# mataiyuan/ASD-SLAM

Hardware: AMD Instinct MI355X
Metric: frames/sec end-to-end tracking+LocalBA, KITTI 00 mono @2000 keypoints (higher is better)
Workload: dtype f32

## Files before the change

asd-slam_amd/capi.py:

```python
import ctypes as C
import os

import numpy as np

_HERE = os.path.dirname(os.path.abspath(__file__))


def lib_path():
    return os.environ.get("ASDHIP_LIB") or os.path.join(_HERE, "libasdhip.so")


class AsdError(RuntimeError):
    def __init__(self, code, msg):
        super().__init__(f"libasdhip error {code}: {msg}")
        self.code = code


class asd_config(C.Structure):
    _fields_ = [("n_features", C.c_int32), ("scale_factor", C.c_float), ("n_levels", C.c_int32),
                ("ini_th_fast", C.c_int32), ("min_th_fast", C.c_int32), ("max_width", C.c_int32),
                ("max_height", C.c_int32), ("max_patches", C.c_int32), ("device", C.c_int32)]


KP_DTYPE = np.dtype([("x", np.float32), ("y", np.float32), ("size", np.float32), ("angle", np.float32),
# ... 72 lines not shown
    frac = np.empty((h, w), np.uint16)
    rc = lib.asd_undistort_map(_p(Kf), _p(df), int(w), int(h), _p(xy), _p(frac))
    if rc != 0:
        raise AsdError(rc, "asd_undistort_map: invalid arguments")
    return xy, frac


def bow_score(scoring, v1, v2):
    lib = load_library()
    lib.asd_last_error.restype = C.c_char_p
    i1, x1, i2, x2 = _c(v1[0], np.int32), _c(v1[1], np.float64), _c(v2[0], np.int32), _c(v2[1], np.float64)
    out = C.c_double(0.0)
    rc = lib.asd_bow_score(int(scoring), len(i1), _p(i1), _p(x1), len(i2), _p(i2), _p(x2), C.byref(out))
    if rc != 0:
        raise AsdError(rc, lib.asd_last_error(None).decode())
    return out.value


class AsdHip:

    def __init__(self, n_features=2000, scale_factor=1.2, n_levels=8, ini_th=20, min_th=7,
                 max_width=1241, max_height=376, max_patches=None, device=0):
        self.lib = load_library()
        L = self.lib
        L.asd_last_error.restype = C.c_char_p
        L.asd_version.restype = C.c_char_p
        L.asd_ctx_stream.restype = C.c_void_p
        self.cfg = asd_config(n_features, scale_factor, n_levels, ini_th, min_th, max_width, max_height,
                              max_patches if max_patches is not None else 2 * n_features, device)
        self.ctx = C.c_void_p()
        rc = L.asd_ctx_create(C.byref(self.cfg), C.byref(self.ctx))
        if rc != 0:
            raise AsdError(rc, "asd_ctx_create failed (no usable HIP device? there is no CPU fallback)")
        self.n_levels = n_levels

    def close(self):
        if getattr(self, "ctx", None) is not None and self.ctx:
            self.lib.asd_ctx_destroy(self.ctx)
            self.ctx = None

    def __del__(self):
        try:
            self.close()
        except Exception:
            pass

    def _chk(self, rc):
        if rc != 0:
            raise AsdError(rc, self.lib.asd_last_error(self.ctx).decode())

    def last_error(self):
        return self.lib.asd_last_error(self.ctx).decode()

    def calibration_note(self):
        self.lib.asd_calibration_note.restype = C.c_char_p
        return self.lib.asd_calibration_note(self.ctx).decode()

    def scale_tables(self):
        n = self.n_levels
        s, i, g, ig = (np.zeros(n, np.float32) for _ in range(4))
        f = np.zeros(n, np.int32)
        self._chk(self.lib.asd_get_scale_tables(self.ctx, _p(s), _p(i), _p(g), _p(ig), _p(f)))
        return dict(scale=s, inv_scale=i, sigma2=g, inv_sigma2=ig, features_per_level=f)

    def load_weights(self, layers, eps=1e-5):
        ws = [_c(w, np.float32) for w, _, _ in layers]
        ms = [_c(m, np.float32) for _, m, _ in layers]
        vs = [_c(v, np.float32) for _, _, v in layers]
        arr = lambda xs: (C.c_void_p * 7)(*[x.ctypes.data for x in xs])
        self._keep = (ws, ms, vs)
        self._chk(self.lib.asd_load_weights(self.ctx, arr(ws), arr(ms), arr(vs), C.c_float(eps)))

    def describe(self, patches):
        patches = _c(patches, np.uint8).reshape(-1, 32, 32)
        n = patches.shape[0]
        out = np.empty((n, 128), np.float32)
        self._chk(self.lib.asd_describe(self.ctx, _p(patches), n, _p(out)))
        return out

    def device_alloc(self, nbytes):
        p = C.c_void_p()
        self._chk(self.lib.asd_device_alloc(self.ctx, C.c_uint64(nbytes), C.byref(p)))
        return p

    def host_alloc(self, nbytes):
        p = C.c_void_p()
        self._chk(self.lib.asd_host_alloc(self.ctx, C.c_uint64(nbytes), C.byref(p)))
        return p

    def device_free(self, p):
        self._chk(self.lib.asd_device_free(self.ctx, p))

    def h2d(self, dptr, arr):
        arr = np.ascontiguousarray(arr)
        self._chk(self.lib.asd_memcpy_h2d(self.ctx, dptr, _p(arr), C.c_uint64(arr.nbytes)))

    def d2h(self, arr, dptr):
        self._chk(self.lib.asd_memcpy_d2h(self.ctx, _p(arr), dptr, C.c_uint64(arr.nbytes)))

    def sync(self):
        self._chk(self.lib.asd_sync(self.ctx))

    def describe_timed(self, d_patches, n, d_desc, reps):
        ms = C.c_float()
        self._chk(self.lib.asd_describe_timed(self.ctx, d_patches, n, d_desc, reps, C.byref(ms)))
        return ms.value

    def debug_act6(self, n):
        out = np.empty((n, 64, 128), np.float32)
        self.lib.asd_debug_act6.argtypes = [C.c_void_p, C.c_int, C.c_void_p]
        self._chk(self.lib.asd_debug_act6(self.ctx, n, _p(out)))
        return out

    def describe_device(self, d_patches, n, d_desc):
        self._chk(self.lib.asd_describe_device(self.ctx, d_patches, n, d_desc))

    def last_stage_ms(self, stage):
        ms = C.c_float()
        self._chk(self.lib.asd_last_stage_ms(self.ctx, stage.encode(), C.byref(ms)))
        return ms.value

    def extract(self, image, n_features_override=0):
        image = np.asarray(image, np.uint8)
        if image.strides[1] != 1 or image.strides[0] < image.shape[1]:
            image = _c(image, np.uint8)
        h, w = image.shape
        cap = self.cfg.max_patches
        kps = np.zeros(cap, KP_DTYPE)
        desc = np.empty((cap, 128), np.float32)
        n = C.c_int32()
        self._chk(self.lib.asd_extract(self.ctx, _p(image), w, h, image.strides[0], n_features_override,
                                       _p(kps), _p(desc), C.byref(n)))
        return kps[:n.value].copy(), desc[:n.value].copy()

    def extract_device(self, d_image, w, h, stride, n_features_override=0):
        cap = self.cfg.max_patches
        if not hasattr(self, "_kps_buf"):
            self._kps_buf = np.zeros(cap, KP_DTYPE)
            self._desc_buf = np.empty((cap, 128), np.float32)
        n = C.c_int32()
        self._chk(self.lib.asd_extract_device(self.ctx, d_image, w, h, stride, n_features_override,
                                              _p(self._kps_buf), _p(self._desc_buf), C.byref(n)))
        return self._kps_buf[:n.value], self._desc_buf[:n.value]

    def extract_submit(self, image, w, h, stride, device_resident=True, n_features_override=0):
        self._chk(self.lib.asd_extract_submit(self.ctx, image, int(device_resident), w, h, stride, n_features_override))

    def extract_wait(self, view=False):
        n = C.c_int32()
        if view:
            pk, pd = C.c_void_p(), C.c_void_p()
            self._chk(self.lib.asd_extract_wait_view(self.ctx, C.byref(pk), C.byref(pd), C.byref(n)))
            if n.value == 0:
                return np.zeros(0, KP_DTYPE), np.zeros((0, 128), np.float32)
            kb = (C.c_char * (n.value * KP_DTYPE.itemsize)).from_address(pk.value)
            db = (C.c_float * (n.value * 128)).from_address(pd.value)
            return np.frombuffer(kb, dtype=KP_DTYPE, count=n.value), np.frombuffer(db, dtype=np.float32).reshape(n.value, 128)
        cap = self.cfg.max_patches
        if not hasattr(self, "_kps_buf"):
            self._kps_buf = np.zeros(cap, KP_DTYPE)
            self._desc_buf = np.empty((cap, 128), np.float32)
        self._chk(self.lib.asd_extract_wait(self.ctx, _p(self._kps_buf), _p(self._desc_buf), C.byref(n)))
        return self._kps_buf[:n.value], self._desc_buf[:n.value]

    def extract_last_view(self):
        self.lib.asd_extract_last_view.restype = C.c_uint64
        return int(self.lib.asd_extract_last_view(self.ctx))

    def extract_view_valid(self, view_id):
        self.lib.asd_extract_view_valid.restype = C.c_int32
        return bool(self.lib.asd_extract_view_valid(self.ctx, C.c_uint64(view_id)))

    def extract_hold(self, on=True):
        self._chk(self.lib.asd_extract_hold(self.ctx, int(on)))

    def set_undistortion(self, K, dist, w, h):
        Kf = None if K is None else _c(K, np.float32)
        df = None if dist is None else _c(dist, np.float32)
        self._chk(self.lib.asd_set_undistortion(self.ctx, _p(Kf), _p(df), int(w), int(h)))

    def undistort(self, image, device_resident=False, w=None, h=None, stride=None):
        if device_resident:
            src = image
        else:
            image = np.asarray(image)
            assert image.dtype == np.uint8 and image.ndim == 2 and image.strides[1] == 1
            h, w = image.shape
            stride = image.strides[0]
            src = C.c_void_p(image.ctypes.data)
        out = np.empty((h, w), np.uint8)
        self._chk(self.lib.asd_undistort(self.ctx, src, int(device_resident), int(w), int(h), int(stride), _p(out), int(w)))
        return out

    def profile_enable(self, on=True):
        self._chk(self.lib.asd_profile_enable(self.ctx, int(on)))

    def profile_get(self, layer):
        ms, calls, patches = C.c_double(), C.c_int32(), C.c_int64()
        self._chk(self.lib.asd_profile_get(self.ctx, layer, C.byref(ms), C.byref(calls), C.byref(patches)))
        return ms.value, calls.value, patches.value

    def asdnet_split_mask(self):
        self.lib.asd_asdnet_split_mask.restype = C.c_int32
        return int(self.lib.asd_asdnet_split_mask(self.ctx))

    def asdnet_pieces(self):
        self.lib.asd_asdnet_pieces.restype = C.c_int32
        return int(self.lib.asd_asdnet_pieces(self.ctx))

    def level_size(self, level):
        w, h = C.c_int32(), C.c_int32()
        self._chk(self.lib.asd_get_level_size(self.ctx, level, C.byref(w), C.byref(h)))
        return w.value, h.value

    def level_image(self, level, blurred=False):
        w, h = self.level_size(level)
        out = np.empty((h, w), np.uint8)
        self._chk(self.lib.asd_get_level_image(self.ctx, level, int(blurred), _p(out)))
        return out

    def raw_corners(self, level, cap=200000):
        x, y, r = (np.empty(cap, np.float32) for _ in range(3))
        n = C.c_int32()
        self._chk(self.lib.asd_get_raw_corners(self.ctx, level, cap, _p(x), _p(y), _p(r), C.byref(n)))
        return x[:n.value].copy(), y[:n.value].copy(), r[:n.value].copy()

    def patches(self):
        cap = self.cfg.max_patches
        out = np.empty((cap, 32, 32), np.uint8)
        n = C.c_int32()
        self._chk(self.lib.asd_get_patches(self.ctx, cap, _p(out), C.byref(n)))
        return out[:n.value].copy()

    def frame_set(self, slot, kps, desc, bounds):
        kps = _c(kps, KP_DTYPE)
        d = None if desc is None else _c(desc, np.float32)
        self._chk(self.lib.asd_frame_set(self.ctx, slot, _p(kps), _p(d), len(kps), C.c_float(bounds[0]),
                                         C.c_float(bounds[1]), C.c_float(bounds[2]), C.c_float(bounds[3])))

    def frame_set_from_ctx(self, slot, kps, bounds, src):
        kps = _c(kps, KP_DTYPE)
        self._chk(self.lib.asd_frame_set_from_ctx(self.ctx, slot, _p(kps), len(kps), C.c_float(bounds[0]), C.c_float(bounds[1]),
                                                  C.c_float(bounds[2]), C.c_float(bounds[3]), src.ctx))

    def extract_keep_pyramid(self, on=True):
        self._chk(self.lib.asd_extract_keep_pyramid(self.ctx, int(on)))

    def features_in_area(self, slot, x, y, r, min_level=-1, max_level=-1, cap=8192):
        out = np.empty(cap, np.int32)
        n = C.c_int32()
        self._chk(self.lib.asd_frame_features_in_area(self.ctx, slot, C.c_float(x), C.c_float(y), C.c_float(r),
                                                      min_level, max_level, cap, _p(out), C.byref(n)))
        return out[:n.value].copy()

    def dist_matrix(self, a, b):
        a, b = _c(a, np.float32), _c(b, np.float32)
        out = np.empty((a.shape[0], b.shape[0]), np.float32)
        self._chk(self.lib.asd_dist_matrix(self.ctx, _p(a), a.shape[0], _p(b), b.shape[0], _p(out)))
        return out

    def distinctive_descriptor(self, desc):
        desc = _c(desc, np.float32)
        best = C.c_int32()
        self._chk(self.lib.asd_distinctive_descriptor(self.ctx, _p(desc), desc.shape[0], C.byref(best)))
        return best.value

    def match_project_frame(self, slot_cur, slot_last, n_cur, has_mp, Xw, mp_desc, Tcw, K, th, check_ori=True, obs_positive=None):
        has_mp, Xw, mp_desc = _c(has_mp, np.uint8), _c(Xw, np.float32), _c(mp_desc, np.float32)
        Tcw, K = _c(Tcw, np.float32), _c(K, np.float32)
        out = np.empty(n_cur, np.int32)
        n = C.c_int32()
        self._chk(self.lib.asd_match_project_frame(self.ctx, slot_cur, slot_last, _p(has_mp), _p(Xw), _p(mp_desc),
                                                   _p(Tcw), _p(K), C.c_float(th), int(check_ori), _p(out),
                                                   C.byref(n), _p(None if obs_positive is None else _c(obs_positive, np.uint8))))
        return out, n.value

    def match_project_points(self, slot_cur, n_cur, in_view, proj, level, view_cos, desc, occupied, th, nn_ratio, obs_positive=None):
        in_view, proj, level = _c(in_view, np.uint8), _c(proj, np.float32), _c(level, np.int32)
        view_cos, desc, occupied = _c(view_cos, np.float32), _c(desc, np.float32), _c(occupied, np.uint8)
        out = np.empty(n_cur, np.int32)
        n = C.c_int32()
        self._chk(self.lib.asd_match_project_points(self.ctx, slot_cur, len(in_view), _p(in_view), _p(proj),
                                                    _p(level), _p(view_cos), _p(desc), _p(occupied), C.c_float(th),
                                                    C.c_float(nn_ratio), _p(out), C.byref(n),
                                                    _p(None if obs_positive is None else _c(obs_positive, np.uint8))))
        return out, n.value

    def track_motion_model(self, slot_cur, slot_last, n_cur, has_mp, Xw, mp_desc_or_rows, Tcw, K, th, pose7, check_ori=True, obs_positive=None, split=False):
        has_mp, Xw, Tcw, K = _c(has_mp, np.uint8), _c(Xw, np.float32), _c(Tcw, np.float32), _c(K, np.float32)
        d = np.asarray(mp_desc_or_rows)
        bank = d.dtype.kind in "iu"
        d = _c(d, np.int32 if bank else np.float32)
        match, outl = np.empty(n_cur, np.int32), np.empty(max(n_cur, 1), np.uint8)
        pose = _c(pose7, np.float64).copy()
        n, ninl = C.c_int32(), C.c_int32()
        fn = self.lib.asd_track_motion_model_bank if bank else self.lib.asd_track_motion_model
        if split:
            self._chk(self.lib.asd_track_async(self.ctx))
        self._chk(fn(self.ctx, slot_cur, slot_last, _p(has_mp), _p(Xw), _p(d), _p(Tcw), _p(K), C.c_float(th), int(check_ori),
                     _p(None if obs_positive is None else _c(obs_positive, np.uint8)), _p(pose), _p(match), C.byref(n), _p(outl), C.byref(ninl)))
        if split:
            self._track_job = (match, n, pose, outl, ninl, n_cur)
            return None
        return match, n.value, pose, outl[:n_cur], ninl.value

    def track_local_map(self, slot_cur, n_cur, in_view, proj, level, view_cos, desc_or_rows, mp_Xw, occupied, cur_Xw, th, nn_ratio, K, pose7,
                        obs_positive=None, split=False):
        in_view, proj, level = _c(in_view, np.uint8), _c(proj, np.float32), _c(level, np.int32)
        view_cos, mp_Xw, occupied, cur_Xw, K = _c(view_cos, np.float32), _c(mp_Xw, np.float32), _c(occupied, np.uint8), _c(cur_Xw, np.float32), _c(K, np.float32)
        d = np.asarray(desc_or_rows)
        bank = d.dtype.kind in "iu"
        d = _c(d, np.int32 if bank else np.float32)
        match, outl = np.empty(n_cur, np.int32), np.empty(max(n_cur, 1), np.uint8)
        pose = _c(pose7, np.float64).copy()
        n, ninl = C.c_int32(), C.c_int32()
        fn = self.lib.asd_track_local_map_bank if bank else self.lib.asd_track_local_map
# ... 475 lines not shown
```

asd-slam_amd/csrc/asdnet.hip:

```cpp
#include "ctx.h"

#include <algorithm>
#include <cmath>
#include <cstring>

typedef float f32x16 __attribute__((ext_vector_type(16)));
typedef float f32x4 __attribute__((ext_vector_type(4)));


namespace {

struct LayerSpec { int cout, cin, k, stride, pad; };
const LayerSpec kLayers[7] = {{32, 1, 3, 1, 1},   {32, 32, 3, 1, 1},   {64, 32, 3, 2, 1},  {64, 64, 3, 1, 1},
                              {128, 64, 3, 2, 1}, {128, 128, 3, 1, 1}, {128, 128, 8, 1, 0}};

template <int CIN, int COUT, int HIN, int S, int ROWS, int WM, int WN, int KC, int PP = 1, int RING = 2>
struct ConvCfg {
  static constexpr int HO = HIN / S;
  static constexpr int INROWS = (ROWS - 1) * S + 3;
  static constexpr int INCOLS = (HO - 1) * S + 3;
  static constexpr int CPAD = CIN + 4;
  static constexpr int NW = WM * WN;
  static constexpr int NTH = 64 * NW;
  static constexpr int M_PATCH = ROWS * HO;
// ... 1180 lines not shown
  const _Float16 hh = (_Float16)xs;
  const _Float16 ll = (_Float16)(xs - (float)hh);
  memcpy(&h, &hh, 2);
  memcpy(&l, &ll, 2);
}

inline float weight_scale_f16(const float* w, size_t count, const std::vector<float>& inv, size_t per_cout) {
  float mx = 0.f;
  for (size_t i = 0; i < count; ++i) mx = std::max(mx, std::fabs(w[i] * inv[i / per_cout]));
  if (!(mx > 0.f) || !std::isfinite(mx)) return 1.f;
  int e;
  (void)std::frexp(mx, &e);
  return std::ldexp(1.f, 14 - e);
}

void build_wx3(const LayerSpec& L, const float* w, const std::vector<float>& inv, std::vector<uint16_t>& img, int np = 3, float wscale = 1.f) {
  img.assign((size_t)9 * L.cin * L.cout * np, 0);
  constexpr int kch = 32, kg = kch / 8;
  const int nc16 = L.cin / kch;
  for (int tap = 0; tap < 9; ++tap)
    for (int ci = 0; ci < L.cin; ++ci)
      for (int co = 0; co < L.cout; ++co) {
        const float v = w[((size_t)co * L.cin + ci) * 9 + tap] * inv[co];
        uint16_t p[3];
        if (np == 3) split3_host(v, p[0], p[1], p[2]);
        else split2_host(v * wscale, p[0], p[1]);
        const int c16 = ci / kch, hh = (ci % kch) / 8, j = ci % 8;
        for (int q = 0; q < np; ++q)
          img[(((((size_t)tap * nc16 + c16) * np + q) * kg + hh) * L.cout + co) * 8 + j] = p[q];
      }
}

void build_wimg(const LayerSpec& L, const float* w, const std::vector<float>& inv, std::vector<float>& img) {
  img.assign((size_t)9 * L.cin * L.cout, 0.f);
  for (int tap = 0; tap < 9; ++tap)
    for (int ci = 0; ci < L.cin; ++ci)
      for (int co = 0; co < L.cout; ++co) {
        const int c8 = ci / 8, hh = (ci % 8) / 4, jj = ci % 4;
        const size_t dst = ((((size_t)tap * (L.cin / 8) + c8) * 2 + hh) * L.cout + co) * 4 + jj;
        img[dst] = w[((size_t)co * L.cin + ci) * 9 + tap] * inv[co];
      }
}

}

int asdnet_alloc(asd_ctx* ctx) {
  const size_t np = (size_t)ctx->cfg.max_patches;
  const size_t npad = (np + 31) / 32 * 32;
  ASD_HIP_CHECK(ctx, hipMalloc(&ctx->d_act[0], np * 32768 * sizeof(float)));
  ASD_HIP_CHECK(ctx, hipMalloc(&ctx->d_act[1], np * 32768 * sizeof(float)));
  ASD_HIP_CHECK(ctx, hipMalloc(&ctx->d_part, (size_t)FC_SK * npad * 128 * sizeof(float)));
  ASD_HIP_CHECK(ctx, hipMalloc(&ctx->d_patches, np * 1024));
  ASD_HIP_CHECK(ctx, hipMalloc(&ctx->d_desc, np * 128 * sizeof(float)));
  ASD_HIP_CHECK(ctx, hipHostMalloc(reinterpret_cast<void**>(&ctx->h_range), 64));
  *ctx->h_range = 0;
  if (const char* e = getenv("ASD_ASDNET_PAIR")) ctx->net_pair = atoi(e) != 0;
  return ASD_OK;
}

void asdnet_free(asd_ctx* ctx) {
  for (int i = 0; i < 2; ++i) if (ctx->d_act[i]) (void)hipFree(ctx->d_act[i]);
  if (ctx->d_part) (void)hipFree(ctx->d_part);
  if (ctx->d_patches) (void)hipFree(ctx->d_patches);
  if (ctx->d_desc) (void)hipFree(ctx->d_desc);
  if (ctx->h_range) (void)hipHostFree(ctx->h_range);
  if (ctx->d_w1) (void)hipFree(ctx->d_w1);
  for (int i = 0; i < 7; ++i) {
    if (ctx->d_bias[i]) (void)hipFree(ctx->d_bias[i]);
    if (ctx->d_wimg[i]) (void)hipFree(ctx->d_wimg[i]);
    if (ctx->d_wx3[i]) (void)hipFree(ctx->d_wx3[i]);
    if (ctx->d_wx2[i]) (void)hipFree(ctx->d_wx2[i]);
  }
}

static int asdnet_calibrate(asd_ctx* ctx, const float* const conv_w[7], const float* const bn_mean[7], const float* const bn_var[7], float eps);

int asdnet_load_weights(asd_ctx* ctx, const float* const conv_w[7], const float* const bn_mean[7],
                        const float* const bn_var[7], float eps) {
  for (int l = 0; l < 7; ++l) {
    const LayerSpec& L = kLayers[l];
    std::vector<float> inv(L.cout), bias(L.cout);
    for (int c = 0; c < L.cout; ++c) {
      inv[c] = 1.0f / std::sqrt(bn_var[l][c] + eps);
      bias[c] = -bn_mean[l][c] * inv[c];
    }
    if (!ctx->d_bias[l]) ASD_HIP_CHECK(ctx, hipMalloc(&ctx->d_bias[l], L.cout * sizeof(float)));
    ASD_HIP_CHECK(ctx, hipMemcpy(ctx->d_bias[l], bias.data(), L.cout * sizeof(float), hipMemcpyHostToDevice));
    std::vector<float> img;
    if (l == 0) {
      img.resize(32 * 9);
      for (int co = 0; co < 32; ++co)
        for (int k = 0; k < 9; ++k) img[co * 9 + k] = conv_w[0][co * 9 + k] * inv[co];
      if (!ctx->d_w1) ASD_HIP_CHECK(ctx, hipMalloc(&ctx->d_w1, img.size() * sizeof(float)));
      ASD_HIP_CHECK(ctx, hipMemcpy(ctx->d_w1, img.data(), img.size() * sizeof(float), hipMemcpyHostToDevice));
      continue;
    }
    if (l < 6) {
      build_wimg(L, conv_w[l], inv, img);
    } else {
      img.assign((size_t)8192 * 128, 0.f);
      for (int px = 0; px < 64; ++px)
        for (int c = 0; c < 128; ++c)
          for (int co = 0; co < 128; ++co) {
            const int k = px * 128 + c, k8 = k / 8, hh = (k % 8) / 4, jj = k % 4;
            img[(((size_t)k8 * 2 + hh) * 128 + co) * 4 + jj] = conv_w[6][((size_t)co * 128 + c) * 64 + px] * inv[co];
          }
    }
    if (!ctx->d_wimg[l]) ASD_HIP_CHECK(ctx, hipMalloc(&ctx->d_wimg[l], img.size() * sizeof(float)));
    ASD_HIP_CHECK(ctx, hipMemcpy(ctx->d_wimg[l], img.data(), img.size() * sizeof(float), hipMemcpyHostToDevice));
    if (l == 6) {
      std::vector<uint16_t> x3((size_t)8192 * 128 * 3, 0);
      for (int px = 0; px < 64; ++px)
        for (int c = 0; c < 128; ++c)
          for (int co = 0; co < 128; ++co) {
            const int k = px * 128 + c, c32 = k / 32, g = (k % 32) / 8, j = k % 8;
            uint16_t pc[3];
            split3_host(conv_w[6][((size_t)co * 128 + c) * 64 + px] * inv[co], pc[0], pc[1], pc[2]);
            for (int q = 0; q < 3; ++q) x3[((((size_t)c32 * 3 + q) * 4 + g) * 128 + co) * 8 + j] = pc[q];
          }
      if (!ctx->d_wx3[l]) ASD_HIP_CHECK(ctx, hipMalloc(&ctx->d_wx3[l], x3.size() * sizeof(uint16_t)));
      ASD_HIP_CHECK(ctx, hipMemcpy(ctx->d_wx3[l], x3.data(), x3.size() * sizeof(uint16_t), hipMemcpyHostToDevice));
      const float ws = weight_scale_f16(conv_w[6], (size_t)128 * 128 * 64, inv, (size_t)128 * 64);
      ctx->wx2_scale[l] = ws;
      std::vector<uint16_t> x2((size_t)8192 * 128 * 2, 0);
      for (int px = 0; px < 64; ++px)
        for (int c = 0; c < 128; ++c)
          for (int co = 0; co < 128; ++co) {
            const int k = px * 128 + c, c32 = k / 32, g = (k % 32) / 8, j = k % 8;
            uint16_t pc[2];
            split2_host(conv_w[6][((size_t)co * 128 + c) * 64 + px] * inv[co] * ws, pc[0], pc[1]);
            for (int q = 0; q < 2; ++q) x2[((((size_t)c32 * 2 + q) * 4 + g) * 128 + co) * 8 + j] = pc[q];
          }
      if (!ctx->d_wx2[l]) ASD_HIP_CHECK(ctx, hipMalloc(&ctx->d_wx2[l], x2.size() * sizeof(uint16_t)));
      ASD_HIP_CHECK(ctx, hipMemcpy(ctx->d_wx2[l], x2.data(), x2.size() * sizeof(uint16_t), hipMemcpyHostToDevice));
    }
    if (l < 6) {
      std::vector<uint16_t> x3;
      build_wx3(L, conv_w[l], inv, x3);
      if (!ctx->d_wx3[l]) ASD_HIP_CHECK(ctx, hipMalloc(&ctx->d_wx3[l], x3.size() * sizeof(uint16_t)));
      ASD_HIP_CHECK(ctx, hipMemcpy(ctx->d_wx3[l], x3.data(), x3.size() * sizeof(uint16_t), hipMemcpyHostToDevice));
      const float ws = weight_scale_f16(conv_w[l], (size_t)L.cout * L.cin * 9, inv, (size_t)L.cin * 9);
      ctx->wx2_scale[l] = ws;
      build_wx3(L, conv_w[l], inv, x3, 2, ws);
      if (!ctx->d_wx2[l]) ASD_HIP_CHECK(ctx, hipMalloc(&ctx->d_wx2[l], x3.size() * sizeof(uint16_t)));
      ASD_HIP_CHECK(ctx, hipMemcpy(ctx->d_wx2[l], x3.data(), x3.size() * sizeof(uint16_t), hipMemcpyHostToDevice));
    }
  }
  ctx->weights_loaded = true;
  return asdnet_calibrate(ctx, conv_w, bn_mean, bn_var, eps);
}

int asdnet_profile_collect_set(asd_ctx* ctx, int set);

static int asdnet_forward_one(asd_ctx* ctx, const uint8_t* d_patches, int n, float* d_desc, hipStream_t st, int* range_flag);
int asdnet_forward_device(asd_ctx* ctx, const uint8_t* d_patches, int n, float* d_desc, hipStream_t st, int* range_flag) {
  if (!ctx->weights_loaded) { ctx->set_error("asd_load_weights has not been called"); return ASD_ERR_NO_WEIGHTS; }
  if (n < 0 || n > ctx->cfg.max_patches) { ctx->set_error("n=%d exceeds max_patches=%d", n, ctx->cfg.max_patches); return ASD_ERR_CAPACITY; }
  if (n == 0) return ASD_OK;
  if (!st) st = ctx->stream;
  std::lock_guard<std::mutex> prof_lock(ctx->prof_mutex);
  return asdnet_forward_one(ctx, d_patches, n, d_desc, st, range_flag);
}
static int asdnet_forward_one(asd_ctx* ctx, const uint8_t* d_patches, int n, float* d_desc, hipStream_t st, int* range_flag) {
  float *a0 = ctx->d_act[0], *a1 = ctx->d_act[1];
  const int npad = (n + 31) / 32 * 32;
  const bool prof = ctx->prof_on;
  const int pset = ctx->prof_cur;
  if (prof && ctx->prof_pending[pset]) { int rc = asdnet_profile_collect_set(ctx, pset); if (rc != ASD_OK) return rc; }
#define PROF_MARK(i) do { if (prof) ASD_HIP_CHECK(ctx, hipEventRecord(ctx->prof_ev[pset][i], st)); } while (0)
  PROF_MARK(0);
  PROF_MARK(1);
#define CALIB(l, buf, elems) do { if (ctx->d_calib) { hipLaunchKernelGGL(k_absmax, dim3(256), dim3(256), 0, st, buf, (size_t)n * (elems), ctx->d_calib + (l)); ASD_HIP_CHECK(ctx, hipGetLastError()); } } while (0)
  ctx->d_act6 = a1;
  if (ctx->net_split) {
    const bool p2 = ctx->net_pieces == 2;
    const bool pair = p2 && ctx->net_pair && !ctx->d_calib;
    const float* x3_stats = nullptr;
#define X3_LAUNCH(CFG, FUSE, l, src, dst, w1p, b1p)                                                                                       \
  (pair ? launch_conv_x3<CFG, FUSE, 2, true>(st, src, ctx->d_wx2[l], ctx->d_bias[l], dst, n, w1p, b1p, nullptr, nullptr, kActScale,          \
                                     1.f / (kActScale * ctx->wx2_scale[l]), x3_stats)                                                               \
   : p2 ? launch_conv_x3<CFG, FUSE, 2>(st, src, ctx->d_wx2[l], ctx->d_bias[l], dst, n, w1p, b1p, nullptr, nullptr, kActScale,               \
                                     1.f / (kActScale * ctx->wx2_scale[l]), x3_stats)                                                               \
      : launch_conv_x3<CFG, FUSE, 3>(st, src, ctx->d_wx3[l], ctx->d_bias[l], dst, n, w1p, b1p, nullptr, nullptr, 1.f, 1.f,                \
                                     x3_stats))
    hipLaunchKernelGGL(k_patch_stats, dim3(n), dim3(256), 0, st, d_patches, ctx->d_part, n);
    ASD_HIP_CHECK(ctx, hipGetLastError());
    x3_stats = ctx->d_part;
    ASD_HIP_CHECK(ctx, (X3_LAUNCH(L2S_CFG, true, 1, d_patches, a1, ctx->d_w1, ctx->d_bias[0])));
    x3_stats = nullptr;
    CALIB(1, a1, 32 * 32 * 32);
    PROF_MARK(2);
    ASD_HIP_CHECK(ctx, (X3_LAUNCH(L3S_CFG, false, 2, a1, a0, nullptr, nullptr)));
    CALIB(2, a0, 16 * 16 * 64);
    PROF_MARK(3);
    ASD_HIP_CHECK(ctx, (X3_LAUNCH(L4S_CFG, false, 3, a0, a1, nullptr, nullptr)));
    CALIB(3, a1, 16 * 16 * 64);
    PROF_MARK(4);
    ASD_HIP_CHECK(ctx, (X3_LAUNCH(L5S_CFG, false, 4, a1, a0, nullptr, nullptr)));
    CALIB(4, a0, 8 * 8 * 128);
    PROF_MARK(5);
    ASD_HIP_CHECK(ctx, (X3_LAUNCH(L6S_CFG, false, 5, a0, a1, nullptr, nullptr)));
#undef X3_LAUNCH
    CALIB(5, a1, 8 * 8 * 128);
    PROF_MARK(6);
    if (pair)
      hipLaunchKernelGGL(k_fc_x2, dim3((npad + FCS_MP - 1) / FCS_MP, FC_SK), dim3(256), 0, st, reinterpret_cast<const uint8_t*>(a1),
                         static_cast<const uint8_t*>(ctx->d_wx2[6]), ctx->d_part, n, npad, 1.f / (kActScale * ctx->wx2_scale[6]));
    else
      hipLaunchKernelGGL(k_fc_x3, dim3((npad + FCS_MP - 1) / FCS_MP, FC_SK), dim3(256), 0, st, a1, static_cast<const uint8_t*>(ctx->d_wx3[6]), ctx->d_part, n, npad);
  } else {
    ASD_HIP_CHECK(ctx, (launch_conv<L2_CFG, true>(st, d_patches, ctx->d_wimg[1], ctx->d_bias[1], a1, n, ctx->d_w1, ctx->d_bias[0])));
    CALIB(1, a1, 32 * 32 * 32);
    PROF_MARK(2);
    ASD_HIP_CHECK(ctx, (launch_conv_p<L3_CFG>(st, a1, ctx->d_wimg[2], ctx->d_bias[2], a0, n, ctx->num_cu)));
    CALIB(2, a0, 16 * 16 * 64);
    PROF_MARK(3);
    ASD_HIP_CHECK(ctx, (launch_conv<L4_CFG>(st, a0, ctx->d_wimg[3], ctx->d_bias[3], a1, n)));
    CALIB(3, a1, 16 * 16 * 64);
    PROF_MARK(4);
    ASD_HIP_CHECK(ctx, (launch_conv<L5_CFG>(st, a1, ctx->d_wimg[4], ctx->d_bias[4], a0, n)));
    CALIB(4, a0, 8 * 8 * 128);
    PROF_MARK(5);
    ASD_HIP_CHECK(ctx, (launch_conv<L6_CFG>(st, a0, ctx->d_wimg[5], ctx->d_bias[5], a1, n)));
    CALIB(5, a1, 8 * 8 * 128);
    PROF_MARK(6);
    hipLaunchKernelGGL(k_fc_mfma, dim3((npad / 32 + FC_MT - 1) / FC_MT, FC_SK), dim3(256), 0, st, a1, ctx->d_wimg[6], ctx->d_part, n, npad);
  }
#undef CALIB
  ASD_HIP_CHECK(ctx, hipGetLastError());
  PROF_MARK(7);
  hipLaunchKernelGGL(k_l2norm, dim3((n + 3) / 4), dim3(256), 0, st, ctx->d_part, ctx->d_bias[6], d_desc, n, npad, range_flag);
  ASD_HIP_CHECK(ctx, hipGetLastError());
  PROF_MARK(8);
#undef PROF_MARK
  if (prof) { ctx->prof_pending[pset] = true; ctx->prof_pending_n[pset] = n; ctx->prof_cur ^= 1; }
  return ASD_OK;
}

static int asdnet_calibrate(asd_ctx* ctx, const float* const conv_w[7], const float* const bn_mean[7], const float* const bn_var[7], float eps) {
  ctx->calib_note.clear();
  ctx->net_pieces = ctx->net_pieces_req;
  if (ctx->net_pieces != 2 || !ctx->net_split) return ASD_OK;
  if (const char* e = getenv("ASD_ASDNET_CALIBRATE")) if (atoi(e) == 0) return ASD_OK;
  const int N = std::min(64, ctx->cfg.max_patches);
  constexpr float kCalibLimit = 2048.f;
  std::vector<uint8_t> pat((size_t)N * 1024);
  uint32_t rng = 0x9e3779b9u;
  auto rnd = [&]() { rng = rng * 1664525u + 1013904223u; return rng >> 8; };
  for (int p = 0; p < N; ++p)
    for (int y = 0; y < 32; ++y)
      for (int x = 0; x < 32; ++x) {
        int v;
        const int kind = p % 8, var = p / 8;
        switch (kind) {
          case 0: v = (int)(rnd() & 255); break;
          case 1: v = (x < 8 + 2 * var) ? 20 : 235; break;
          case 2: v = (y < 8 + 2 * var) ? 235 : 20; break;
          case 3: v = (x + y < 24 + 2 * var) ? 10 : 245; break;
          case 4: v = (((x >> (var % 3)) + (y >> (var % 3))) & 1) ? 255 : 0; break;
          case 5: v = (x * 255) / 31; break;
          case 6: v = (x == 4 * var + 1 && y == 3 * var + 2) ? 255 : 0; break;
          default: v = 128 + (int)(rnd() & 3); break;
        }
        pat[(size_t)p * 1024 + y * 32 + x] = (uint8_t)v;
      }
  float max1 = 0.f;
  {
    std::vector<float> inv(32), bias(32);
    for (int c = 0; c < 32; ++c) { inv[c] = 1.0f / std::sqrt(bn_var[0][c] + eps); bias[c] = -bn_mean[0][c] * inv[c]; }
    std::vector<float> in(34 * 34);
    for (int p = 0; p < N; ++p) {
      double s1 = 0, s2 = 0;
      for (int i = 0; i < 1024; ++i) s1 += pat[(size_t)p * 1024 + i] / 255.0;
      const double mean = s1 / 1024;
      for (int i = 0; i < 1024; ++i) { const double d = pat[(size_t)p * 1024 + i] / 255.0 - mean; s2 += d * d; }
      const double sd = std::sqrt(s2 / 1023) + 1e-7;
      std::fill(in.begin(), in.end(), 0.f);
      for (int y = 0; y < 32; ++y)
        for (int x = 0; x < 32; ++x) in[(y + 1) * 34 + x + 1] = (float)((pat[(size_t)p * 1024 + y * 32 + x] / 255.0 - mean) / sd);
      for (int c = 0; c < 32; ++c)
        for (int y = 0; y < 32; ++y)
          for (int x = 0; x < 32; ++x) {
            float a = bias[c];
            for (int k = 0; k < 9; ++k) a += in[(y + k / 3) * 34 + x + k % 3] * conv_w[0][c * 9 + k] * inv[c];
            max1 = std::max(max1, a);
          }
    }
  }
  uint8_t* d_pat = nullptr;
  unsigned* d_max = nullptr;
  float* d_out = nullptr;
  int rc = ASD_OK;
  unsigned hmax[8] = {};
  do {
    if (hipMalloc(&d_pat, pat.size()) != hipSuccess || hipMalloc(&d_max, 8 * sizeof(unsigned)) != hipSuccess ||
        hipMalloc(&d_out, (size_t)N * 128 * sizeof(float)) != hipSuccess) { rc = ASD_ERR_HIP; break; }
    if (hipMemcpy(d_pat, pat.data(), pat.size(), hipMemcpyHostToDevice) != hipSuccess || hipMemset(d_max, 0, 8 * sizeof(unsigned)) != hipSuccess) { rc = ASD_ERR_HIP; break; }
    ctx->d_calib = d_max;
    rc = asdnet_forward_device(ctx, d_pat, N, d_out, ctx->stream, nullptr);
    ctx->d_calib = nullptr;
    if (rc != ASD_OK) break;
    if (hipStreamSynchronize(ctx->stream) != hipSuccess || hipMemcpy(hmax, d_max, sizeof hmax, hipMemcpyDeviceToHost) != hipSuccess) rc = ASD_ERR_HIP;
  } while (0);
  if (d_pat) (void)hipFree(d_pat);
  if (d_max) (void)hipFree(d_max);
  if (d_out) (void)hipFree(d_out);
  if (rc != ASD_OK) { ctx->set_error("asd_load_weights: the range calibration pass failed"); return rc; }
  float worst = max1;
  int worst_layer = 1;
  for (int l = 1; l <= 5; ++l) {
    float v;
    memcpy(&v, &hmax[l], 4);
    if (!(v <= 3.0e38f)) v = INFINITY;
    if (v > worst) { worst = v; worst_layer = l + 1; }
  }
  if (worst > kCalibLimit) {
    ctx->net_pieces = 3;
    char buf[256];
    snprintf(buf, sizeof buf, "asd_load_weights: calibration found |activation| = %g behind conv%d (limit %g for the two-piece fp16 form): this context uses the three-piece bf16 form (asd_asdnet_pieces = 3)",
             (double)worst, worst_layer, (double)kCalibLimit);
    ctx->calib_note = buf;
  }
  return ASD_OK;
}

int asdnet_profile_collect_set(asd_ctx* ctx, int set) {
  if (!ctx->prof_pending[set]) return ASD_OK;
  ASD_HIP_CHECK(ctx, hipEventSynchronize(ctx->prof_ev[set][8]));
  for (int l = 0; l < 8; ++l) {
    float ms = 0;
    ASD_HIP_CHECK(ctx, hipEventElapsedTime(&ms, ctx->prof_ev[set][l], ctx->prof_ev[set][l + 1]));
    ctx->prof_ms[l] += ms;
    ctx->prof_calls[l] += 1;
    ctx->prof_patches[l] += ctx->prof_pending_n[set];
  }
  ctx->prof_pending[set] = false;
  return ASD_OK;
}

int asdnet_profile_collect(asd_ctx* ctx) {
// ... 69 lines not shown
```

asd-slam_amd/csrc/ctx.h:

```cpp
#pragma once
#include <hip/hip_runtime.h>

#include <atomic>
#include <cstdarg>
#include <cstdio>
#include <cstdlib>
#include <cstring>
#include <functional>
#include <mutex>
#include <string>
#include <vector>

#include "../../include/asd_slam.h"

#define ASD_HIP_CHECK(ctx, expr)                                                          \
  do {                                                                                    \
    hipError_t _e = (expr);                                                               \
    if (_e != hipSuccess) {                                                               \
      (ctx)->set_error("%s failed: %s (%s:%d)", #expr, hipGetErrorString(_e), __FILE__, __LINE__); \
      return ASD_ERR_HIP;                                                                 \
    }                                                                                     \
  } while (0)

struct AsdPerDeviceOnce {
// ... 82 lines not shown
      int lvl = 0;
      for (int k = 1; k < a.n_levels; ++k) lvl += ratio >= a.level_thr[k];
      float r = vc > 0.998 ? 2.5f : 4.0f;
      if (a.bfactor) r *= a.th;
      Q = AsdWinQuery{u, v, r * a.scale[lvl], lvl - 1, lvl, row};
    }
  }
  a.queries[q] = Q;
}
__device__ inline void asd_between_body(const AsdBetweenArgs& a_dev, const int t, const int nt) {
#pragma clang fp contract(off)
  const AsdBetweenArgs a = a_dev;
  __shared__ int s_nmatch;
  if (t == 0) s_nmatch = 0;
  for (int c = t; c < a.n_cand; c += nt) a.skip[c] = 0;
  asd_syncthreads();
  const uint8_t* outl = reinterpret_cast<const uint8_t*>(a.io1 + 8);
  int mine = 0;
  for (int j = t; j < a.n_cur; j += nt) {
    const int i = a.match1[j];
    mine += i >= 0;
    const int src = i >= 0 ? i : 0;
    for (int k = 0; k < 3; ++k) a.cur_Xw[3 * (size_t)j + k] = a.n_last > 0 ? a.Xw_last[3 * (size_t)src + k] : 0.f;
    const bool keep = i >= 0 && !outl[j];
    a.occ[j] = keep ? 1 : 0;
    if (i >= 0 && a.last_cand) { const int c = a.last_cand[i]; if (c >= 0 && c < a.n_cand) a.skip[c] = 1; }
  }
  if (mine) atomicAdd(&s_nmatch, mine);
  asd_syncthreads();
  if (t == 0) {
    float T[16];
    if (s_nmatch >= 3) {
      const double* p = a.io1;
      const double x = p[0], y = p[1], z = p[2], w = p[3];
      const double tx = 2 * x, ty = 2 * y, tz = 2 * z;
      const double twx = tx * w, twy = ty * w, twz = tz * w, txx = tx * x, txy = ty * x, txz = tz * x, tyy = ty * y, tyz = tz * y, tzz = tz * z;
      const double R[9] = {1 - (tyy + tzz), txy - twz, txz + twy, txy + twz, 1 - (txx + tzz), tyz - twx, txz - twy, tyz + twx, 1 - (txx + tyy)};
      for (int i = 0; i < 3; ++i) {
        for (int j = 0; j < 3; ++j) T[i * 4 + j] = (float)R[i * 3 + j];
        T[i * 4 + 3] = (float)p[4 + i];
      }
      T[12] = T[13] = T[14] = 0.f;
      T[15] = 1.f;
    } else {
      for (int i = 0; i < 16; ++i) T[i] = a.T_pred[i];
    }
    for (int i = 0; i < 16; ++i) a.T1[i] = T[i];
    for (int i = 0; i < 3; ++i) {
      double sum = 0;
      for (int k = 0; k < 3; ++k) sum += (double)T[k * 4 + i] * (double)T[k * 4 + 3];
      a.T1[16 + i] = (float)(-1.0 * sum);
    }
  }
}
#endif

struct AsdXfer {
  char* h = nullptr;
  char* d = nullptr;
  size_t cap = 0, used = 0;
  hipError_t begin(hipStream_t st, size_t bytes) {
    used = 0;
    bytes += 4096;
    if (bytes <= cap) return hipSuccess;
    if (h) { (void)hipStreamSynchronize(st); (void)hipHostFree(h); (void)hipFree(d); }
    h = nullptr; d = nullptr; cap = 0;
    const size_t want = bytes + bytes / 2;
    hipError_t e = hipHostMalloc(&h, want);
    if (e == hipSuccess) e = hipMalloc(&d, want);
    if (e == hipSuccess) cap = want;
    return e;
  }
  size_t reserve(size_t bytes) { const size_t off = used; used += (bytes + 255) / 256 * 256; return off; }
  size_t add(const void* src, size_t bytes) { const size_t off = reserve(bytes); memcpy(h + off, src, bytes); return off; }
  size_t zeros(size_t bytes) { const size_t off = reserve(bytes); memset(h + off, 0, bytes); return off; }
  hipError_t upload(hipStream_t st) {
    if (!used) return hipSuccess;
    static const bool by_kernel = getenv("ASD_UPLOAD_COPY") == nullptr;
    return by_kernel ? asd_copy_rows(st, d, h, (used + 15) / 16 * 16) : hipMemcpyAsync(d, h, used, hipMemcpyHostToDevice, st);
  }
  hipError_t download(hipStream_t st) { return used ? hipMemcpyAsync(h, d, used, hipMemcpyDeviceToHost, st) : hipSuccess; }
  template <typename T> T* dev(size_t off) { return reinterpret_cast<T*>(d + off); }
  template <typename T> T* host(size_t off) { return reinterpret_cast<T*>(h + off); }
  void release() { if (h) (void)hipHostFree(h); if (d) (void)hipFree(d); h = d = nullptr; cap = used = 0; }
};

struct AsdFrameSlot {
  int n = 0;
  float min_x = 0, max_x = 0, min_y = 0, max_y = 0;
  float inv_w = 0, inv_h = 0;
  std::vector<asd_keypoint> kps;
  std::vector<int32_t> cell_start;
  std::vector<int32_t> cell_items;
  float* d_desc = nullptr;
  float4* d_kp = nullptr;
  int32_t* d_cell_start = nullptr;
  int32_t* d_cell_items = nullptr;
  int32_t* d_fv = nullptr;
  int32_t fv_nodes = 0;
  char* h_stage = nullptr;
  hipEvent_t ev_staged = nullptr;
};

struct UndistortMap {
  int w = 0, h = 0, mpitch = 0;
  short2* d_xy = nullptr;
  uint16_t* d_frac = nullptr;
  uint8_t* d_io = nullptr;
};

struct asd_ctx {
  asd_config cfg{};
  hipStream_t stream = nullptr;
  hipStream_t stream_x = nullptr;
  hipStream_t stream_prep = nullptr;
  hipEvent_t ev_prep = nullptr;
  bool prep_on = false;
  struct AsyncExtract* ax = nullptr;
  int num_cu = 256;
  std::string err;

  float scale[ASD_MAX_LEVELS], inv_scale[ASD_MAX_LEVELS], sigma2[ASD_MAX_LEVELS], inv_sigma2[ASD_MAX_LEVELS];
  int features_per_level[ASD_MAX_LEVELS];
  float level_thr[ASD_MAX_LEVELS];
  int umax[16];

  bool weights_loaded = false;
  float* d_w1 = nullptr;
  float* d_bias[7] = {};
  float* d_wimg[7] = {};
  void* d_wx3[7] = {};
  bool match_replay_host = false;
  bool ba_struct_host = false;
  void* d_wx2[7] = {};
  float wx2_scale[7] = {1, 1, 1, 1, 1, 1, 1};
  int net_pieces_req = 2;
  int net_pieces = 2;
  int net_split = 0x3f;
  float* d_act[2] = {};
  float* d_part = nullptr;
  int* h_range = nullptr;
  std::string calib_note;
  unsigned* d_calib = nullptr;
  bool pose_chain_kp_flags = false;
  bool net_pair = true;
  float* d_act6 = nullptr;
  uint8_t* d_patches = nullptr;
  int patches_n = 0;
  float* d_desc = nullptr;
  bool keep_pyramid = false;
  const uint8_t* d_pyr_view = nullptr;
  AsdDevBuf stereo_scratch;
  float* d_desc_last = nullptr;
  hipEvent_t ev_adopt = nullptr;
  bool adopt_pending = false;

  struct FrontendState* fe = nullptr;
  UndistortMap* und = nullptr;
  int last_n = 0;

  AsdFrameSlot frames[ASD_MAX_FRAMES];

  void* matcher = nullptr;

  void* ba = nullptr;

  AsdDevBuf scratch;
  AsdXfer up, down;
  bool track_async_armed = false, track_has_pending = false;
  hipEvent_t ev_chain = nullptr;
  std::function<int()> track_pending;

  void* mapping = nullptr;

  void* bow = nullptr;

  void* sim3 = nullptr;

  void* kfdb = nullptr;

  std::mutex prof_mutex;
  bool prof_on = false;
  hipEvent_t prof_ev[2][9] = {};
  bool prof_pending[2] = {false, false};
  int prof_pending_n[2] = {0, 0};
  int prof_cur = 0;
  double prof_ms[8] = {};
  int prof_calls[8] = {};
  long long prof_patches[8] = {};

  hipEvent_t ev0 = nullptr, ev1 = nullptr, ev2 = nullptr;
  float ms_asdnet = 0, ms_extract = 0, ms_match = 0, ms_ba = 0, ms_sim3 = 0, ms_kfdb = 0;

  std::mutex err_mutex;
  std::string err_returned;
  void set_error(const char* fmt, ...) {
    char buf[512];
    va_list ap;
    va_start(ap, fmt);
    vsnprintf(buf, sizeof buf, fmt, ap);
    va_end(ap);
    std::lock_guard<std::mutex> l(err_mutex);
    err = buf;
  }
  const char* last_error() {
    std::lock_guard<std::mutex> l(err_mutex);
    err_returned = err;
    return err_returned.c_str();
  }
};

inline hipStream_t asd_prep_stream(asd_ctx* ctx) { return ctx->prep_on ? ctx->stream_prep : ctx->stream; }

int frontend_alloc(asd_ctx* ctx);
void frontend_free(asd_ctx* ctx);
void frontend_async_shutdown(asd_ctx* ctx);
bool asd_extractor_busy(asd_ctx* ctx, const char* who);
int frontend_image_to_device(asd_ctx* ctx, const uint8_t* image, bool on_device, int width, int height, int stride, uint8_t* dst,
                             int pitch, hipStream_t st);
int undistort_launch(asd_ctx* ctx, const UndistortMap& U, hipStream_t st, const uint8_t* src, int stride, uint8_t* dst, int pitch);
void undistort_free(asd_ctx* ctx);
bool asd_track_busy(asd_ctx* ctx, const char* who);
void matcher_free(asd_ctx* ctx);
void ba_free(asd_ctx* ctx);
void mapping_free(asd_ctx* ctx);
void bow_free(asd_ctx* ctx);
void sim3_free(asd_ctx* ctx);
void kfdb_free(asd_ctx* ctx);
const char* kfdb_host_error();
struct AsdFusedReplay { const void* args; int kind; int nq; size_t lds; };
bool pose_chain_fused_ok(const asd_ctx* ctx, int kind, int nq, int n_cur, size_t lds);
int pose_chain_enqueue(asd_ctx* ctx, int n_cur, const int* d_src, const float4* d_kp, const float* d_tab, const uint8_t* d_hold,
                       const float* d_own, const double* pose7, const double* K, double* d_io, const double* d_pose0 = nullptr,
                       double* d_io_dev = nullptr, const AsdBetweenArgs* between = nullptr, const AsdFusedReplay* fused = nullptr);
int pose_chain_reserve(asd_ctx* ctx, int n_cur);
inline bool pose_chain_lds_form(const asd_ctx* ctx, int n_cur) { return ctx->cfg.n_levels <= 16 && (size_t)n_cur * 35 + 16 <= 150 * 1024; }
inline size_t pose_chain_io_bytes(int n_cur) { return 64 + ((size_t)n_cur + 7) / 8 * 8 + 64; }
void asd_compute_quotas(int nfeatures, float scaleFactor, int nl, int* out);

inline int asd_range_status(asd_ctx* ctx, int* flag, const char* who) {
  if (!flag || !*flag) return ASD_OK;
  *flag = 0;
  ctx->set_error("%s: an ASDNet activation left the range of the two-piece fp16 operand form (|x| > 4094): the descriptors of this call are "
                 "not valid.  ASD_ASDNET_MATH=bf16x3 (or f32) has no range limit", who);
  return ASD_ERR_RANGE;
}
int asdnet_alloc(asd_ctx* ctx);
void asdnet_free(asd_ctx* ctx);
int asdnet_load_weights(asd_ctx* ctx, const float* const conv_w[7], const float* const bn_mean[7],
                        const float* const bn_var[7], float eps);
int asdnet_forward_device(asd_ctx* ctx, const uint8_t* d_patches, int n, float* d_desc, hipStream_t st, int* range_flag = nullptr);
int asdnet_profile_collect(asd_ctx* ctx);
```

asd-slam_amd/csrc/frontend.hip:

```cpp
#include <algorithm>
#include <cfloat>
#include <cmath>
#include <cstring>

#include <atomic>
#include <chrono>
#include <condition_variable>
#include <functional>
#include <map>
#include <mutex>
#include <thread>

#include "ctx.h"
#include "quadtree.h"

namespace {

constexpr int kEdge = 19;
constexpr int kMinBorder = 16;
constexpr int kPitchAlign = 64;

inline int cv_round(double v) { return (int)std::lrint(v); }
inline int cv_floor(double v) { return (int)std::floor(v); }
inline short sat_short(float v) { int i = cv_round(v); return (short)std::min(std::max(i, -32768), 32767); }
// ... 99 lines not shown
  }
}

template <bool WRITE>
__global__ __launch_bounds__(64) void k_cell_nms(const CellDev* __restrict__ cells, PyrDev P,
                                                 const uint8_t* __restrict__ score, int ini_th,
                                                 int* __restrict__ cell_count, const int* __restrict__ cell_off,
                                                 uint32_t* __restrict__ out, int out_cap) {
  const CellDev c = cells[blockIdx.x];
  const LevelDev& L = P.lv[c.level];
  const uint8_t* S = score + L.off;
  const int cw = c.x1 - c.x0, chh = c.y1 - c.y0, area = cw * chh;
  const int lane = threadIdx.x;
  int n20 = 0, n7 = 0;
  bool use20 = false;
  int base = 0;
  if (WRITE) {
    const int cnt = cell_count[blockIdx.x];
    use20 = cnt < 0;
    base = cell_off[blockIdx.x];
  }
  for (int i0 = 0; i0 < area; i0 += 64) {
    const int i = i0 + lane;
    bool keep = false, is20 = false;
    int x = 0, y = 0, s = 0;
    if (i < area) {
      x = c.x0 + i % cw;
      y = c.y0 + i / cw;
      s = S[(size_t)y * L.pitch + x];
      if (s > 0) {
        keep = true;
        for (int dy = -1; dy <= 1; ++dy)
          for (int dx = -1; dx <= 1; ++dx) {
            if (dx == 0 && dy == 0) continue;
            const int xx = x + dx, yy = y + dy;
            if (xx < c.x0 || xx >= c.x1 || yy < c.y0 || yy >= c.y1) continue;
            if (S[(size_t)yy * L.pitch + xx] >= s) keep = false;
          }
        is20 = keep && s >= ini_th;
      }
    }
    if (!WRITE) {
      n20 += __popcll(__ballot(is20));
      n7 += __popcll(__ballot(keep));
    } else {
      const bool w = use20 ? is20 : keep;
      const unsigned long long m = __ballot(w);
      if (w) {
        const int pos = base + __popcll(m & ((1ull << lane) - 1));
        if (pos < out_cap) out[pos] = (uint32_t)(x - kMinBorder) | ((uint32_t)(y - kMinBorder) << 12) | ((uint32_t)s << 24);
      }
      base += __popcll(m);
    }
  }
  if (!WRITE && lane == 0) cell_count[blockIdx.x] = n20 > 0 ? (n20 | 0x80000000) : n7;
}

__global__ __launch_bounds__(1024) void k_cell_scan(const int* __restrict__ cell_count, int ncells,
                                                    const int* __restrict__ level_cell_start, int nlevels,
                                                    int* __restrict__ cell_off, int* __restrict__ level_start,
                                                    int* __restrict__ level_start_host) {
  __shared__ int wsum[16];
  __shared__ int carry_s;
  const int t = threadIdx.x, lane = t & 63, wave = t >> 6;
  if (t == 0) carry_s = 0;
  asd_syncthreads();
  for (int base = 0; base < ncells; base += 1024) {
    const int i = base + t;
    const int v = i < ncells ? (cell_count[i] & 0x7fffffff) : 0;
    int incl = v;
    for (int off = 1; off < 64; off <<= 1) {
      const int o = __shfl_up(incl, off);
      if (lane >= off) incl += o;
    }
    if (lane == 63) wsum[wave] = incl;
    asd_syncthreads();
    int wbase = 0;
    for (int w = 0; w < wave; ++w) wbase += wsum[w];
    const int carry = carry_s;
    if (i < ncells) cell_off[i] = carry + wbase + incl - v;
    asd_syncthreads();
    if (t == 1023) carry_s = carry + wbase + incl;
    asd_syncthreads();
  }
  if (t <= nlevels) {
    int v;
    if (t == nlevels) v = carry_s;
    else {
      const int c = level_cell_start[t];
      v = c < ncells ? cell_off[c] : carry_s;
    }
    level_start[t] = v;
    level_start_host[t] = v;
  }
}

__device__ inline int reflect101(int p, int len) {
  if (p < 0) p = -p;
  if (p >= len) p = 2 * len - 2 - p;
  return p;
}
__global__ __launch_bounds__(256) void k_blur7(PyrDev P, const uint8_t* __restrict__ pyr, uint8_t* __restrict__ blur) {
  __shared__ int rows[22][64];
  int local;
  const LevelDev& L = find_level(P, blockIdx.x, local);
  const int x = (local % L.tiles_x) * 64 + (threadIdx.x & 63);
  const int y0 = (local / L.tiles_x) * 16;
  const uint8_t* img = pyr + L.off;
  const int wq = threadIdx.x >> 6;
  const int xc = min(x, L.w - 1);
  int xs[7];
  for (int i = 0; i < 7; ++i) xs[i] = reflect101(xc + i - 3, L.w);
  for (int r = wq; r < 22; r += 4) {
    const int yy = reflect101(min(y0 + r - 3, L.h + 2), L.h);
    const uint8_t* row = img + (size_t)yy * L.pitch;
    int s = 0;
    for (int i = 0; i < 7; ++i) s += c_gauss[i] * row[xs[i]];
    rows[r][threadIdx.x & 63] = s;
  }
  asd_syncthreads();
  for (int r = wq; r < 16; r += 4) {
    const int yy = y0 + r;
    if (yy >= L.h || x >= L.w) continue;
    int s = 0;
    for (int i = 0; i < 7; ++i) s += c_gauss[i] * rows[r + i][threadIdx.x & 63];
    const int v = (s + (1 << 15)) >> 16;
    blur[L.off + (size_t)yy * L.pitch + x] = (uint8_t)min(max(v, 0), 255);
  }
}

__device__ inline float fast_atan2_deg(float y, float x) {
  const float p1 = 0.9997878412794807f * (float)(180 / M_PI);
  const float p3 = -0.3258083974640975f * (float)(180 / M_PI);
  const float p5 = 0.1555786518463281f * (float)(180 / M_PI);
  const float p7 = -0.04432655554792128f * (float)(180 / M_PI);
  const float ax = fabsf(x), ay = fabsf(y);
  float a, c, c2;
  if (ax >= ay) {
    c = ay / (ax + (float)DBL_EPSILON);
    c2 = c * c;
    a = (((p7 * c2 + p5) * c2 + p3) * c2 + p1) * c;
  } else {
    c = ax / (ay + (float)DBL_EPSILON);
    c2 = c * c;
    a = 90.f - (((p7 * c2 + p5) * c2 + p3) * c2 + p1) * c;
  }
  if (x < 0) a = 180.f - a;
  if (y < 0) a = 360.f - a;
  return a;
}

__global__ __launch_bounds__(256) void k_angle_patch(PyrDev P, const uint8_t* __restrict__ pyr,
                                                     const uint8_t* __restrict__ blur, const short4* __restrict__ kps,
                                                     int n, float* __restrict__ angles, uint8_t* __restrict__ patches) {
  const int lane = threadIdx.x & 63;
  const int k = blockIdx.x * 4 + (threadIdx.x >> 6);
  if (k >= n) return;
  const short4 kp = kps[k];
  const LevelDev& L = P.lv[kp.z];
  const uint8_t* center = pyr + L.off + (size_t)kp.y * L.pitch + kp.x;
  int m01 = 0, m10 = 0;
  for (int i = lane; i < c_ndisc; i += 64) {
    const short2 o = c_disc[i];
    const int val = center[o.y * L.pitch + o.x];
    m10 += o.x * val;
    m01 += o.y * val;
  }
  for (int off = 32; off >= 1; off >>= 1) {
    m01 += __shfl_xor(m01, off);
    m10 += __shfl_xor(m10, off);
  }
  if (lane == 0) angles[k] = fast_atan2_deg((float)m01, (float)m10);
  const int row = lane >> 1, half = lane & 1;
  const uint8_t* src = blur + L.off + (size_t)(kp.y - 16 + row) * L.pitch + (kp.x - 16 + half * 16);
  uint32_t w[4];
  for (int q = 0; q < 4; ++q)
    w[q] = (uint32_t)src[q * 4] | ((uint32_t)src[q * 4 + 1] << 8) | ((uint32_t)src[q * 4 + 2] << 16) |
           ((uint32_t)src[q * 4 + 3] << 24);
  *reinterpret_cast<uint4*>(patches + (size_t)k * 1024 + row * 32 + half * 16) = make_uint4(w[0], w[1], w[2], w[3]);
}


class LevelPool {
 public:
  explicit LevelPool(int nworkers) {
    for (int i = 0; i < nworkers; ++i) th_.emplace_back([this] { worker(); });
  }
  ~LevelPool() {
    { std::lock_guard<std::mutex> l(m_); stop_ = true; ++gen_; }
    cv_.notify_all();
    for (auto& t : th_) t.join();
  }
  void run(int ntasks, const std::function<void(int)>& job) {
    {
      std::lock_guard<std::mutex> l(m_);
      job_ = &job; ntasks_ = ntasks; next_.store(0); active_ = (int)th_.size(); ++gen_;
    }
    cv_.notify_all();
    drain();
    std::unique_lock<std::mutex> l(m_);
    done_cv_.wait(l, [this] { return active_ == 0; });
    job_ = nullptr;
  }
 private:
  void drain() {
    for (;;) {
      const int i = next_.fetch_add(1);
      if (i >= ntasks_) break;
      (*job_)(i);
    }
  }
  void worker() {
    unsigned long long seen = 0;
    for (;;) {
      {
        std::unique_lock<std::mutex> l(m_);
        cv_.wait(l, [&] { return gen_ != seen; });
        seen = gen_;
        if (stop_) return;
      }
      drain();
      { std::lock_guard<std::mutex> l(m_); --active_; }
      done_cv_.notify_one();
    }
  }
  std::vector<std::thread> th_;
  std::mutex m_;
  std::condition_variable cv_, done_cv_;
  const std::function<void(int)>* job_ = nullptr;
  std::atomic<int> next_{0};
  int ntasks_ = 0, active_ = 0;
  unsigned long long gen_ = 0;
  bool stop_ = false;
};

}

struct ExtractSlot {
  uint8_t* d_patches = nullptr;
  float* d_desc = nullptr;
  float *d_angles = nullptr, *h_angles = nullptr, *h_desc = nullptr;
  int* h_range = nullptr;
  hipEvent_t ev_begin = nullptr, ev_front = nullptr, ev_end = nullptr;
  bool owned = false;
  uint8_t* d_pyr_keep = nullptr;
  size_t pyr_keep_cap = 0;
};

struct FrontendState {
  int cfg_w = 0, cfg_h = 0;
  PyrDev pyr{};
  size_t buf_bytes = 0;
  uint8_t *d_pyr = nullptr, *d_blur = nullptr, *d_score = nullptr;
  short *d_xofs = nullptr, *d_ialpha = nullptr, *d_yofs = nullptr, *d_ibeta = nullptr;
  int tab_x_off[ASD_MAX_LEVELS] = {}, tab_y_off[ASD_MAX_LEVELS] = {};
  size_t tab_x_cap = 0, tab_y_cap = 0;
  std::vector<CellDev> h_cells;
  int level_cell_start[ASD_MAX_LEVELS + 1] = {};
  CellDev* d_cells = nullptr;
  int cells_cap = 0;
  int *d_cell_count = nullptr, *d_cell_off = nullptr, *d_level_cell_start = nullptr, *d_level_start = nullptr;
  size_t corners_cap = 0;
  uint32_t* h_corners = nullptr;
  int* h_level_start = nullptr;
  short4 *d_kps = nullptr, *h_kps = nullptr;
  float *d_angles = nullptr, *h_angles = nullptr, *h_desc = nullptr;
  std::vector<float> raw_x[ASD_MAX_LEVELS], raw_y[ASD_MAX_LEVELS], raw_r[ASD_MAX_LEVELS];
  std::vector<int> sel[ASD_MAX_LEVELS];
  LevelPool* pool = nullptr;
  uint8_t* d_stage = nullptr;
  int stage_pitch = 0;
  ExtractSlot slot0;
};

static void level_dims(const asd_ctx* ctx, int w, int h, int level, int* lw, int* lh) {
  const float s = ctx->inv_scale[level];
  *lw = cv_round((float)w * s);
  *lh = cv_round((float)h * s);
}

static int fe_alloc(asd_ctx* ctx, FrontendState** out) {
  FrontendState* fe = new FrontendState();
  *out = fe;
  fe->pool = new LevelPool(3);
  const int nl = ctx->cfg.n_levels, W = ctx->cfg.max_width, H = ctx->cfg.max_height;
  size_t bytes = 0, tx = 0, ty = 0;
  int ncell_max = 0;
  for (int l = 0; l < nl; ++l) {
    int lw, lh;
    level_dims(ctx, W, H, l, &lw, &lh);
    const int pitch = (lw + kPitchAlign - 1) / kPitchAlign * kPitchAlign;
    bytes += (size_t)pitch * (lh + 1);
    tx += lw; ty += lh;
    ncell_max += (lw / 30 + 2) * (lh / 30 + 2);
  }
  fe->buf_bytes = bytes + 4096;
  fe->stage_pitch = (W + kPitchAlign - 1) / kPitchAlign * kPitchAlign;
  ASD_HIP_CHECK(ctx, hipMalloc(&fe->d_pyr, fe->buf_bytes));
  ASD_HIP_CHECK(ctx, hipMalloc(&fe->d_blur, fe->buf_bytes));
  ASD_HIP_CHECK(ctx, hipMalloc(&fe->d_score, fe->buf_bytes));
  fe->tab_x_cap = tx + 64; fe->tab_y_cap = ty + 64;
  ASD_HIP_CHECK(ctx, hipMalloc(&fe->d_xofs, fe->tab_x_cap * sizeof(short)));
  ASD_HIP_CHECK(ctx, hipMalloc(&fe->d_ialpha, fe->tab_x_cap * 2 * sizeof(short)));
  ASD_HIP_CHECK(ctx, hipMalloc(&fe->d_yofs, fe->tab_y_cap * sizeof(short)));
  ASD_HIP_CHECK(ctx, hipMalloc(&fe->d_ibeta, fe->tab_y_cap * 2 * sizeof(short)));
  fe->cells_cap = ncell_max;
  ASD_HIP_CHECK(ctx, hipMalloc(&fe->d_cells, ncell_max * sizeof(CellDev)));
  ASD_HIP_CHECK(ctx, hipMalloc(&fe->d_cell_count, ncell_max * sizeof(int)));
  ASD_HIP_CHECK(ctx, hipMalloc(&fe->d_cell_off, ncell_max * sizeof(int)));
  ASD_HIP_CHECK(ctx, hipMalloc(&fe->d_level_cell_start, (ASD_MAX_LEVELS + 1) * sizeof(int)));
  ASD_HIP_CHECK(ctx, hipMalloc(&fe->d_level_start, (ASD_MAX_LEVELS + 1) * sizeof(int)));
  fe->corners_cap = bytes / 4 + 1024;
  ASD_HIP_CHECK(ctx, hipHostMalloc(&fe->h_corners, fe->corners_cap * sizeof(uint32_t)));
  ASD_HIP_CHECK(ctx, hipHostMalloc(&fe->h_level_start, (ASD_MAX_LEVELS + 1) * sizeof(int)));
  const size_t np = ctx->cfg.max_patches;
  ASD_HIP_CHECK(ctx, hipMalloc(&fe->d_kps, np * sizeof(short4)));
  ASD_HIP_CHECK(ctx, hipHostMalloc(&fe->h_kps, np * sizeof(short4)));
  ASD_HIP_CHECK(ctx, hipMalloc(&fe->d_angles, np * sizeof(float)));
  ASD_HIP_CHECK(ctx, hipHostMalloc(&fe->h_angles, (np + 16) * sizeof(float)));
  ASD_HIP_CHECK(ctx, hipHostMalloc(&fe->h_desc, np * 128 * sizeof(float)));
  return ASD_OK;
}
int frontend_alloc(asd_ctx* ctx) { return fe_alloc(ctx, &ctx->fe); }

static void fe_free(FrontendState* fe) {
  if (!fe) return;
  void* dev[] = {fe->d_pyr, fe->d_blur, fe->d_score, fe->d_xofs, fe->d_ialpha, fe->d_yofs, fe->d_ibeta, fe->d_cells,
                 fe->d_cell_count, fe->d_cell_off, fe->d_level_cell_start, fe->d_level_start,
                 fe->d_kps, fe->d_angles, fe->d_stage};
  for (void* p : dev) if (p) (void)hipFree(p);
  void* host[] = {fe->h_corners, fe->h_level_start, fe->h_kps, fe->h_angles, fe->h_desc};
  for (void* p : host) if (p) (void)hipHostFree(p);
  for (hipEvent_t* e : {&fe->slot0.ev_begin, &fe->slot0.ev_front, &fe->slot0.ev_end})
    if (*e) (void)hipEventDestroy(*e);
  delete fe->pool;
  delete fe;
}
void frontend_free(asd_ctx* ctx) { fe_free(ctx->fe); ctx->fe = nullptr; }

static int configure_size(asd_ctx* ctx, FrontendState* fe, int w, int h) {
  if (fe->cfg_w == w && fe->cfg_h == h) return ASD_OK;
  const int nl = ctx->cfg.n_levels;
  static std::mutex consts_mu;
  static AsdPerDeviceOnce consts_once;
  std::lock_guard<std::mutex> consts_lock(consts_mu);
  if (consts_once.need(ctx->cfg.device)) {
    int gk[7];
    float cf[7];
    double sum = 0;
    for (int i = 0; i < 7; i++) { const double x = i - 3.0; cf[i] = (float)std::exp(-0.5 / 4.0 * x * x); sum += cf[i]; }
    sum = 1. / sum;
    for (int i = 0; i < 7; i++) { cf[i] = (float)(cf[i] * sum); gk[i] = cv_round(cf[i] * 256.f); }
    ASD_HIP_CHECK(ctx, hipMemcpyToSymbol(HIP_SYMBOL(c_gauss), gk, sizeof gk));
    std::vector<short2> disc;
    for (int v = -15; v <= 15; ++v) {
      const int d = ctx->umax[v < 0 ? -v : v];
      for (int u = -d; u <= d; ++u) disc.push_back(make_short2((short)u, (short)v));
    }
    const int nd = (int)disc.size();
    if (nd > 768) { ctx->set_error("orientation disc has %d pixels", nd); return ASD_ERR_INVALID; }
    ASD_HIP_CHECK(ctx, hipMemcpyToSymbol(HIP_SYMBOL(c_disc), disc.data(), nd * sizeof(short2)));
    ASD_HIP_CHECK(ctx, hipMemcpyToSymbol(HIP_SYMBOL(c_ndisc), &nd, sizeof nd));
    consts_once.done(ctx->cfg.device);
  }
  PyrDev& P = fe->pyr;
  fe->cfg_w = fe->cfg_h = 0;
  P.nlevels = nl;
  int off = 0, tiles = 0;
  size_t tx = 0, ty = 0;
  for (int l = 0; l < nl; ++l) {
    LevelDev& L = P.lv[l];
    level_dims(ctx, w, h, l, &L.w, &L.h);
    if (L.w < 2 * kEdge + 8 || L.h < 2 * kEdge + 8) { ctx->set_error("image %dx%d too small for level %d", w, h, l); return ASD_ERR_INVALID; }
    L.pitch = (L.w + kPitchAlign - 1) / kPitchAlign * kPitchAlign;
    L.off = off;
    off += L.pitch * L.h;
    L.tiles_x = (L.w + 63) / 64;
    L.tile_start = tiles;
    tiles += L.tiles_x * ((L.h + 15) / 16);
    fe->tab_x_off[l] = (int)tx; fe->tab_y_off[l] = (int)ty;
    tx += L.w; ty += L.h;
  }
  P.total_tiles = tiles;
  if ((size_t)off > fe->buf_bytes || tx > fe->tab_x_cap || ty > fe->tab_y_cap) { ctx->set_error("image %dx%d exceeds ctx capacity", w, h); return ASD_ERR_CAPACITY; }
  std::vector<short> xofs(tx), ialpha(tx * 2), yofs(ty), ibeta(ty * 2);
  for (int l = 1; l < nl; ++l) {
    const int sw = P.lv[l - 1].w, sh = P.lv[l - 1].h, dw = P.lv[l].w, dh = P.lv[l].h;
    const double inv_scale_x = (double)dw / sw, inv_scale_y = (double)dh / sh;
    const double scale_x = 1. / inv_scale_x, scale_y = 1. / inv_scale_y;
    for (int dx = 0; dx < dw; dx++) {
      float fx = (float)((dx + 0.5) * scale_x - 0.5);
      int sx = cv_floor(fx);
      fx -= sx;
      if (sx < 0) { fx = 0; sx = 0; }
      if (sx >= sw - 1) { fx = 0; sx = sw - 1; }
      const size_t o = fe->tab_x_off[l] + dx;
      xofs[o] = (short)sx;
      ialpha[o * 2] = sat_short((1.f - fx) * 2048);
      ialpha[o * 2 + 1] = sat_short(fx * 2048);
    }
    for (int dy = 0; dy < dh; dy++) {
      float fy = (float)((dy + 0.5) * scale_y - 0.5);
      const int sy = cv_floor(fy);
      fy -= sy;
      const size_t o = fe->tab_y_off[l] + dy;
      yofs[o] = (short)sy;
      ibeta[o * 2] = sat_short((1.f - fy) * 2048);
      ibeta[o * 2 + 1] = sat_short(fy * 2048);
    }
  }
  ASD_HIP_CHECK(ctx, hipMemcpy(fe->d_xofs, xofs.data(), tx * sizeof(short), hipMemcpyHostToDevice));
  ASD_HIP_CHECK(ctx, hipMemcpy(fe->d_ialpha, ialpha.data(), tx * 2 * sizeof(short), hipMemcpyHostToDevice));
  ASD_HIP_CHECK(ctx, hipMemcpy(fe->d_yofs, yofs.data(), ty * sizeof(short), hipMemcpyHostToDevice));
  ASD_HIP_CHECK(ctx, hipMemcpy(fe->d_ibeta, ibeta.data(), ty * 2 * sizeof(short), hipMemcpyHostToDevice));
  fe->h_cells.clear();
  for (int l = 0; l < nl; ++l) {
    fe->level_cell_start[l] = (int)fe->h_cells.size();
    const LevelDev& L = P.lv[l];
    const int minBX = kMinBorder, minBY = kMinBorder, maxBX = L.w - kEdge + 3, maxBY = L.h - kEdge + 3;
    const float width = (float)(maxBX - minBX), height = (float)(maxBY - minBY);
    const int nCols = (int)(width / 30.f), nRows = (int)(height / 30.f);
    if (nCols < 1 || nRows < 1) continue;
    const int wCell = (int)std::ceil(width / nCols), hCell = (int)std::ceil(height / nRows);
    for (int i = 0; i < nRows; i++) {
      const float iniY = (float)(minBY + i * hCell);
      float maxY = iniY + hCell + 6;
      if (iniY >= maxBY - 3) continue;
      if (maxY > maxBY) maxY = (float)maxBY;
      for (int j = 0; j < nCols; j++) {
        const float iniX = (float)(minBX + j * wCell);
        float maxX = iniX + wCell + 6;
        if (iniX >= maxBX - 6) continue;
        if (maxX > maxBX) maxX = (float)maxBX;
        const int cw = (int)maxX - (int)iniX, ch = (int)maxY - (int)iniY;
        if (cw < 7 || ch < 7) continue;
        CellDev c;
        c.level = (short)l;
        c.x0 = (short)((int)iniX + 3); c.x1 = (short)((int)maxX - 3);
        c.y0 = (short)((int)iniY + 3); c.y1 = (short)((int)maxY - 3);
        c.pad = 0;
        fe->h_cells.push_back(c);
      }
    }
  }
  fe->level_cell_start[nl] = (int)fe->h_cells.size();
  for (int l = nl + 1; l <= ASD_MAX_LEVELS; ++l) fe->level_cell_start[l] = (int)fe->h_cells.size();
  if ((int)fe->h_cells.size() > fe->cells_cap) { ctx->set_error("cell table overflow"); return ASD_ERR_CAPACITY; }
  ASD_HIP_CHECK(ctx, hipMemcpy(fe->d_cells, fe->h_cells.data(), fe->h_cells.size() * sizeof(CellDev), hipMemcpyHostToDevice));
  ASD_HIP_CHECK(ctx, hipMemcpy(fe->d_level_cell_start, fe->level_cell_start, (ASD_MAX_LEVELS + 1) * sizeof(int), hipMemcpyHostToDevice));
  fe->cfg_w = w; fe->cfg_h = h;
  return ASD_OK;
}

struct ExtractJob {
  const uint8_t* image = nullptr;
  bool on_device = false;
  int w = 0, h = 0, stride = 0, nfeat = 0;
  int n = 0, rc = ASD_OK;
};

static int slot_alloc(asd_ctx* ctx, ExtractSlot& S) {
  const size_t np = ctx->cfg.max_patches;
  ASD_HIP_CHECK(ctx, hipMalloc(&S.d_patches, np * 1024));
  ASD_HIP_CHECK(ctx, hipMalloc(&S.d_desc, np * 128 * sizeof(float)));
  ASD_HIP_CHECK(ctx, hipMalloc(&S.d_angles, np * sizeof(float)));
  ASD_HIP_CHECK(ctx, hipHostMalloc(&S.h_angles, (np + 16) * sizeof(float)));
  S.h_range = reinterpret_cast<int*>(S.h_angles + np);
  ASD_HIP_CHECK(ctx, hipHostMalloc(&S.h_desc, np * 128 * sizeof(float)));
  S.owned = true;
  return ASD_OK;
}
static int slot_events(asd_ctx* ctx, ExtractSlot& S) {
  if (!S.ev_begin) ASD_HIP_CHECK(ctx, hipEventCreate(&S.ev_begin));
  if (!S.ev_front) ASD_HIP_CHECK(ctx, hipEventCreate(&S.ev_front));
  if (!S.ev_end) ASD_HIP_CHECK(ctx, hipEventCreate(&S.ev_end));
  return ASD_OK;
}
static void slot_free(ExtractSlot& S) {
  if (S.owned) {
    if (S.d_patches) (void)hipFree(S.d_patches);
    if (S.d_desc) (void)hipFree(S.d_desc);
    if (S.d_angles) (void)hipFree(S.d_angles);
    if (S.h_angles) (void)hipHostFree(S.h_angles);
    if (S.h_desc) (void)hipHostFree(S.h_desc);
  }
  for (hipEvent_t* e : {&S.ev_begin, &S.ev_front, &S.ev_end})
    if (*e) { (void)hipEventDestroy(*e); *e = nullptr; }
  if (S.d_pyr_keep) (void)hipFree(S.d_pyr_keep);
  S = ExtractSlot();
}

int frontend_image_to_device(asd_ctx* ctx, const uint8_t* image, bool on_device, int width, int height, int stride, uint8_t* dst,
                             int pitch, hipStream_t st) {
  bool by_kernel = on_device;
  const uint8_t* src_dev = image;
  if (!by_kernel) {
    hipPointerAttribute_t at{};
    by_kernel = hipPointerGetAttributes(&at, image) == hipSuccess && at.type == hipMemoryTypeHost && at.devicePointer != nullptr;
    if (!by_kernel) (void)hipGetLastError();
    else src_dev = static_cast<const uint8_t*>(at.devicePointer) + (image - static_cast<const uint8_t*>(at.hostPointer ? at.hostPointer : image));
  }
  if (by_kernel) {
    hipLaunchKernelGGL(k_copy_image, dim3((width + 1023) / 1024, height), dim3(256), 0, st, src_dev, stride, width, height, dst, pitch);
    ASD_HIP_CHECK(ctx, hipGetLastError());
  } else {
    ASD_HIP_CHECK(ctx, hipMemcpy2DAsync(dst, pitch, image, stride, width, height, hipMemcpyHostToDevice, st));
  }
  return ASD_OK;
}

static int extract_front(asd_ctx* ctx, FrontendState* fe, const ExtractJob& J, ExtractSlot& S, hipStream_t st, hipEvent_t ev_corners,
                         asd_keypoint* kps, int32_t* n_out) {
  const int width = J.w, height = J.h, stride = J.stride;
  int rc = configure_size(ctx, fe, width, height);
  if (rc != ASD_OK) return rc;
  const PyrDev& P = fe->pyr;
  const int nl = P.nlevels;
  int quota[ASD_MAX_LEVELS];
  const int nfeat = J.nfeat > 0 ? J.nfeat : ctx->cfg.n_features;
  if (nfeat > ctx->cfg.max_patches) { ctx->set_error("n_features %d exceeds max_patches", nfeat); return ASD_ERR_CAPACITY; }
  if (J.nfeat > 0) asd_compute_quotas(nfeat, ctx->cfg.scale_factor, nl, quota);
  else for (int l = 0; l < nl; ++l) quota[l] = ctx->features_per_level[l];

  const bool timing = getenv("ASD_TIMING") != nullptr;
  auto now = [] { return std::chrono::steady_clock::now(); };
  auto us = [](std::chrono::steady_clock::time_point a, std::chrono::steady_clock::time_point b) { return std::chrono::duration<double, std::micro>(b - a).count(); };
  const auto t_start = now();
  ASD_HIP_CHECK(ctx, hipEventRecord(S.ev_begin, st));
  if (!ctx->und) {
    if ((rc = frontend_image_to_device(ctx, J.image, J.on_device, width, height, stride, fe->d_pyr + P.lv[0].off, P.lv[0].pitch, st)) != ASD_OK) return rc;
  } else {
    const uint8_t* src = J.image;
    int src_stride = stride;
    if (!J.on_device) {
      if (!fe->d_stage) ASD_HIP_CHECK(ctx, hipMalloc(&fe->d_stage, (size_t)fe->stage_pitch * ctx->cfg.max_height));
      if ((rc = frontend_image_to_device(ctx, J.image, false, width, height, stride, fe->d_stage, fe->stage_pitch, st)) != ASD_OK) return rc;
      src = fe->d_stage; src_stride = fe->stage_pitch;
    }
    if ((rc = undistort_launch(ctx, *ctx->und, st, src, src_stride, fe->d_pyr + P.lv[0].off, P.lv[0].pitch)) != ASD_OK) return rc;
  }
  for (int l = 1; l < nl; ++l) {
    const LevelDev &Sl = P.lv[l - 1], &D = P.lv[l];
    hipLaunchKernelGGL(k_resize, dim3((D.w + 255) / 256, (D.h + 3) / 4), dim3(256), 0, st, fe->d_pyr + Sl.off, Sl.w, Sl.h,
                       Sl.pitch, fe->d_pyr + D.off, D.w, D.h, D.pitch, fe->d_xofs + fe->tab_x_off[l],
                       fe->d_ialpha + 2 * fe->tab_x_off[l], fe->d_yofs + fe->tab_y_off[l],
                       fe->d_ibeta + 2 * fe->tab_y_off[l]);
  }
  if (ctx->keep_pyramid) {
    size_t bytes = 0;
    for (int l = 0; l < nl; ++l) bytes = std::max(bytes, (size_t)P.lv[l].off + (size_t)P.lv[l].pitch * P.lv[l].h);
    bytes = (bytes + 15) / 16 * 16;
    if (S.pyr_keep_cap < fe->buf_bytes) {
      if (S.d_pyr_keep) (void)hipFree(S.d_pyr_keep);
      S.d_pyr_keep = nullptr; S.pyr_keep_cap = 0;
      ASD_HIP_CHECK(ctx, hipMalloc(&S.d_pyr_keep, fe->buf_bytes));
      S.pyr_keep_cap = fe->buf_bytes;
    }
    ASD_HIP_CHECK(ctx, asd_copy_rows(st, S.d_pyr_keep, fe->d_pyr, bytes));
  }
  const int ncells = (int)fe->h_cells.size();
  hipLaunchKernelGGL(k_fast_score, dim3(P.total_tiles), dim3(256), 0, st, P, fe->d_pyr, fe->d_score, ctx->cfg.min_th_fast);
  hipLaunchKernelGGL(k_cell_nms<false>, dim3(ncells), dim3(64), 0, st, fe->d_cells, P, fe->d_score, ctx->cfg.ini_th_fast,
                     fe->d_cell_count, fe->d_cell_off, fe->h_corners, 0);
  hipLaunchKernelGGL(k_cell_scan, dim3(1), dim3(1024), 0, st, fe->d_cell_count, ncells, fe->d_level_cell_start, nl,
                     fe->d_cell_off, fe->d_level_start, fe->h_level_start);
  hipLaunchKernelGGL(k_cell_nms<true>, dim3(ncells), dim3(64), 0, st, fe->d_cells, P, fe->d_score, ctx->cfg.ini_th_fast,
                     fe->d_cell_count, fe->d_cell_off, fe->h_corners, (int)fe->corners_cap);
  ASD_HIP_CHECK(ctx, hipGetLastError());
  ASD_HIP_CHECK(ctx, hipEventRecord(ev_corners, st));
  hipLaunchKernelGGL(k_blur7, dim3(P.total_tiles), dim3(256), 0, st, P, fe->d_pyr, fe->d_blur);
  ASD_HIP_CHECK(ctx, hipGetLastError());
  ASD_HIP_CHECK(ctx, hipEventSynchronize(ev_corners));
  const auto t_counts = now();
  const int total = fe->h_level_start[nl];
  if ((size_t)total > fe->corners_cap) { ctx->set_error("corner buffer overflow"); return ASD_ERR_CAPACITY; }
  const auto t_corners = now();
  const std::function<void(int)> level_job = [&](int l) {
    const int b = fe->h_level_start[l], e = fe->h_level_start[l + 1], cnt = e - b;
    auto &rx = fe->raw_x[l], &ry = fe->raw_y[l], &rr = fe->raw_r[l];
    rx.resize(cnt); ry.resize(cnt); rr.resize(cnt);
    for (int i = 0; i < cnt; ++i) {
      const uint32_t pk = fe->h_corners[b + i];
      rx[i] = (float)(pk & 0xfff);
      ry[i] = (float)((pk >> 12) & 0xfff);
      rr[i] = (float)(pk >> 24);
    }
    const LevelDev& L = P.lv[l];
    asd_distribute_octtree(rx.data(), ry.data(), rr.data(), cnt, kMinBorder, L.w - kEdge + 3, kMinBorder,
                           L.h - kEdge + 3, quota[l], fe->sel[l]);
  };
  fe->pool->run(nl, level_job);
  int n = 0;
  for (int l = 0; l < nl; ++l) {
    auto &rx = fe->raw_x[l], &ry = fe->raw_y[l], &rr = fe->raw_r[l];
    const int scaledPatchSize = (int)(31 * ctx->scale[l]);
    for (int idx : fe->sel[l]) {
      if (n >= ctx->cfg.max_patches) { ctx->set_error("more keypoints than max_patches"); return ASD_ERR_CAPACITY; }
      const float px = rx[idx] + kMinBorder, py = ry[idx] + kMinBorder;
      fe->h_kps[n] = make_short4((short)px, (short)py, (short)l, 0);
      asd_keypoint& k = kps[n];
      k.x = px; k.y = py;
      if (l != 0) { k.x *= ctx->scale[l]; k.y *= ctx->scale[l]; }
      k.size = (float)scaledPatchSize;
      k.response = rr[idx];
      k.octave = l;
      k.angle = 0.f;
      ++n;
    }
  }
  *n_out = n;
  const auto t_quad = now();
  if (n > 0) {
    ASD_HIP_CHECK(ctx, hipMemcpyAsync(fe->d_kps, fe->h_kps, (size_t)n * sizeof(short4), hipMemcpyHostToDevice, st));
    hipLaunchKernelGGL(k_angle_patch, dim3((n + 3) / 4), dim3(256), 0, st, P, fe->d_pyr, fe->d_blur, fe->d_kps, n,
                       S.d_angles, S.d_patches);
    ASD_HIP_CHECK(ctx, hipGetLastError());
    ASD_HIP_CHECK(ctx, hipMemcpyAsync(S.h_angles, S.d_angles, (size_t)n * sizeof(float), hipMemcpyDeviceToHost, st));
  }
  ASD_HIP_CHECK(ctx, hipEventRecord(S.ev_front, st));
  if (timing) fprintf(stderr, "[extract front] launch+counts %.0f us, corners D2H %.0f us (%d), quadtree %.0f us\n", us(t_start, t_counts), us(t_counts, t_corners), total, us(t_corners, t_quad));
  return ASD_OK;
}

static int extract_back_enqueue(asd_ctx* ctx, ExtractSlot& S, int n, hipStream_t st) {
  ASD_HIP_CHECK(ctx, hipStreamWaitEvent(st, S.ev_front, 0));
  if (S.h_range) *S.h_range = 0;
  const int rc = asdnet_forward_device(ctx, S.d_patches, n, S.d_desc, st, S.h_range);
  if (rc != ASD_OK) return rc;
  ASD_HIP_CHECK(ctx, hipMemcpyAsync(S.h_desc, S.d_desc, (size_t)n * 128 * sizeof(float), hipMemcpyDeviceToHost, st));
  ASD_HIP_CHECK(ctx, hipEventRecord(S.ev_end, st));
  return ASD_OK;
}

static int extract_finish(asd_ctx* ctx, ExtractSlot& S, int n, asd_keypoint* kps, float* desc) {
  ASD_HIP_CHECK(ctx, hipEventSynchronize(S.ev_end));
  if (desc) memcpy(desc, S.h_desc, (size_t)n * 128 * sizeof(float));
  for (int i = 0; i < n; ++i) kps[i].angle = S.h_angles[i];
  ASD_HIP_CHECK(ctx, hipEventElapsedTime(&ctx->ms_extract, S.ev_begin, S.ev_end));
  return asd_range_status(ctx, S.h_range, "asd_extract");
}

static int extract_check(asd_ctx* ctx, const uint8_t* image, int32_t width, int32_t height, int32_t stride) {
  if (!ctx || !image) return ASD_ERR_INVALID;
  if (width < 1 || height < 1 || stride < width) { ctx->set_error("image %dx%d with stride %d: stride < width or an empty image", width, height, stride); return ASD_ERR_INVALID; }
  if (width > ctx->cfg.max_width || height > ctx->cfg.max_height) { ctx->set_error("image %dx%d exceeds ctx capacity %dx%d", width, height, ctx->cfg.max_width, ctx->cfg.max_height); return ASD_ERR_CAPACITY; }
  if (!ctx->weights_loaded) { ctx->set_error("asd_load_weights has not been called"); return ASD_ERR_NO_WEIGHTS; }
  if (ctx->und && (width != ctx->und->w || height != ctx->und->h)) {
    ctx->set_error("image %dx%d, the undistortion map (asd_set_undistortion) is %dx%d", width, height, ctx->und->w, ctx->und->h);
    return ASD_ERR_INVALID;
  }
  return ASD_OK;
}

extern "C" {

static int extract_impl(asd_ctx* ctx, const uint8_t* image, bool image_on_device, int32_t width, int32_t height,
                        int32_t stride, int32_t n_features_override, asd_keypoint* kps, float* desc, int32_t* n_out) {
  if (!kps || !desc || !n_out) return ASD_ERR_INVALID;
  int rc = extract_check(ctx, image, width, height, stride);
  if (rc != ASD_OK) return rc;
  if (asd_extractor_busy(ctx, "asd_extract")) return ASD_ERR_INVALID;
  (void)hipSetDevice(ctx->cfg.device);
  ctx->adopt_pending = false;
  FrontendState* fe = ctx->fe;
  ExtractSlot& S = fe->slot0;
  if (!S.d_patches) {
    S.d_patches = ctx->d_patches; S.d_desc = ctx->d_desc;
    S.d_angles = fe->d_angles; S.h_angles = fe->h_angles; S.h_desc = fe->h_desc;
    S.h_range = reinterpret_cast<int*>(fe->h_angles + ctx->cfg.max_patches);
  }
  if ((rc = slot_events(ctx, S)) != ASD_OK) return rc;
  ExtractJob J;
  J.image = image; J.on_device = image_on_device; J.w = width; J.h = height; J.stride = stride; J.nfeat = n_features_override;
  int32_t n = 0;
  ctx->patches_n = 0;
  if ((rc = extract_front(ctx, fe, J, S, ctx->stream, ctx->ev2, kps, &n)) != ASD_OK) return rc;
  *n_out = n;
  ctx->patches_n = n;
  ctx->last_n = n;
  ctx->d_desc_last = S.d_desc;
  ctx->d_pyr_view = nullptr;
  if (n == 0) return ASD_OK;
  if ((rc = extract_back_enqueue(ctx, S, n, ctx->stream)) != ASD_OK) return rc;
  return extract_finish(ctx, S, n, kps, desc);
}

int asd_extract(asd_ctx* ctx, const uint8_t* image, int32_t width, int32_t height, int32_t stride,
                int32_t n_features_override, asd_keypoint* kps, float* desc, int32_t* n_out) {
  return extract_impl(ctx, image, false, width, height, stride, n_features_override, kps, desc, n_out);
}

int asd_extract_device(asd_ctx* ctx, const uint8_t* d_image, int32_t width, int32_t height, int32_t stride,
                       int32_t n_features_override, asd_keypoint* kps, float* desc, int32_t* n_out) {
  return extract_impl(ctx, d_image, true, width, height, stride, n_features_override, kps, desc, n_out);
}

}

constexpr int kQueueDepth = ASD_EXTRACT_QUEUE;
constexpr int kSlots = kQueueDepth + 2;

struct AsyncJob {
  ExtractJob job;
  int slot = 0;
  enum State { QUEUED, FRONT, BACK, DONE } state = QUEUED;
  std::vector<asd_keypoint> kps;
};

constexpr int kWorkers = 2;
struct AsyncExtract {
  std::thread th[kWorkers];
  std::mutex m;
  std::condition_variable cv;
  bool stop = false;
  hipStream_t stream_f[kWorkers] = {};
  hipEvent_t ev_corners[kWorkers] = {};
  FrontendState* fe[kWorkers] = {};
  ExtractSlot slots[kSlots];
  AsyncJob jobs[kSlots];
  uint64_t submitted = 0, started = 0, waited = 0;
  uint64_t back_next = 0;
  bool hold_back = false;
  uint64_t last_view = ~0ull;
};

static void async_worker(asd_ctx* ctx, int wk) {
  AsyncExtract* ax = ctx->ax;
  (void)hipSetDevice(ctx->cfg.device);
  static const bool timing = getenv("ASD_TIMING") != nullptr;
  double t_idle = 0, t_front = 0, t_back = 0;
  long jobs = 0;
  for (;;) {
    AsyncJob* next = nullptr;
    uint64_t seq = 0;
    const auto w0 = std::chrono::steady_clock::now();
    {
      std::unique_lock<std::mutex> l(ax->m);
      ax->cv.wait(l, [&] { return ax->stop || ax->started < ax->submitted; });
      if (ax->stop) return;
      seq = ax->started;
      next = &ax->jobs[seq % kSlots];
      ++ax->started;
      next->state = AsyncJob::FRONT;
    }
    const auto w1 = std::chrono::steady_clock::now();
    ExtractSlot& S = ax->slots[next->slot];
    int32_t n = 0;
    int rc = extract_front(ctx, ax->fe[wk], next->job, S, ax->stream_f[wk], ax->ev_corners[wk], next->kps.data(), &n);
    const auto w2 = std::chrono::steady_clock::now();
    next->job.n = n;
    {
      std::unique_lock<std::mutex> l(ax->m);
      ax->cv.wait(l, [&] { return ax->stop || (ax->back_next == seq && !ax->hold_back); });
      if (ax->stop) return;
    }
    if (rc == ASD_OK && n > 0) rc = extract_back_enqueue(ctx, S, n, ctx->stream_x);
    if (timing) {
      const auto w3 = std::chrono::steady_clock::now();
      auto us = [](auto a, auto b) { return std::chrono::duration<double, std::micro>(b - a).count(); };
      t_idle += us(w0, w1); t_front += us(w1, w2); t_back += us(w2, w3);
      if (++jobs % 100 == 0) fprintf(stderr, "[extract worker %d] per frame: waiting for a job %.0f us, front half %.0f us, back half (turn + enqueue) %.0f us\n", wk, t_idle / jobs, t_front / jobs, t_back / jobs);
    }
    {
      std::lock_guard<std::mutex> l(ax->m);
      next->job.rc = rc;
      next->state = (rc != ASD_OK || n == 0) ? AsyncJob::DONE : AsyncJob::BACK;
      ++ax->back_next;
    }
    ax->cv.notify_all();
  }
}

void frontend_async_shutdown(asd_ctx* ctx) {
  if (!ctx->ax) return;
  AsyncExtract* ax = ctx->ax;
  { std::lock_guard<std::mutex> l(ax->m); ax->stop = true; }
  ax->cv.notify_all();
  for (auto& th : ax->th) if (th.joinable()) th.join();
  if (ctx->stream_x) (void)hipStreamSynchronize(ctx->stream_x);
  for (hipStream_t st : ax->stream_f) if (st) (void)hipStreamSynchronize(st);
  for (auto& S : ax->slots) slot_free(S);
  for (hipEvent_t e : ax->ev_corners) if (e) (void)hipEventDestroy(e);
  for (hipStream_t st : ax->stream_f) if (st) (void)hipStreamDestroy(st);
  for (int w = 1; w < kWorkers; ++w) fe_free(ax->fe[w]);
  delete ax;
  ctx->ax = nullptr;
  if (ctx->stream_x) (void)hipStreamDestroy(ctx->stream_x);
  ctx->stream_x = nullptr;
}

bool asd_extractor_busy(asd_ctx* ctx, const char* who) {
  AsyncExtract* ax = ctx->ax;
  if (!ax) return false;
  std::lock_guard<std::mutex> l(ax->m);
  if (ax->submitted == ax->waited) return false;
  ctx->set_error("%s: %llu submission(s) of asd_extract_submit are outstanding -- the worker thread owns the pyramid, score and "
                 "activation buffers until asd_extract_wait has returned them all", who, (unsigned long long)(ax->submitted - ax->waited));
  return true;
}

extern "C" {

int asd_extract_hold(asd_ctx* ctx, int32_t on) {
  if (!ctx) return ASD_ERR_INVALID;
  AsyncExtract* ax = ctx->ax;
  if (!ax) return ASD_OK;
  { std::lock_guard<std::mutex> l(ax->m); ax->hold_back = on != 0; }
  ax->cv.notify_all();
  return ASD_OK;
}

int asd_extract_submit(asd_ctx* ctx, const uint8_t* image, int32_t device_resident, int32_t width, int32_t height,
                       int32_t stride, int32_t n_features_override) {
  int rc = extract_check(ctx, image, width, height, stride);
  if (rc != ASD_OK) return rc;
  (void)hipSetDevice(ctx->cfg.device);
  if (!ctx->ax) {
    int prio_least = 0, prio_greatest = 0;
    (void)hipDeviceGetStreamPriorityRange(&prio_least, &prio_greatest);
    AsyncExtract* ax = new AsyncExtract();
    hipStream_t sx = nullptr;
    auto build = [&]() -> int {
      ASD_HIP_CHECK(ctx, hipStreamCreateWithPriority(&sx, hipStreamDefault, prio_least));
      ax->fe[0] = ctx->fe;
      for (int w = 0; w < kWorkers; ++w) {
        ASD_HIP_CHECK(ctx, hipStreamCreateWithPriority(&ax->stream_f[w], hipStreamDefault, prio_greatest));
        ASD_HIP_CHECK(ctx, hipEventCreate(&ax->ev_corners[w]));
        int r;
        if (w > 0 && (r = fe_alloc(ctx, &ax->fe[w])) != ASD_OK) return r;
      }
      for (int i = 0; i < kSlots; ++i) {
        int r;
        if ((r = slot_alloc(ctx, ax->slots[i])) != ASD_OK) return r;
        if ((r = slot_events(ctx, ax->slots[i])) != ASD_OK) return r;
        ax->jobs[i].slot = i;
        ax->jobs[i].kps.resize(ctx->cfg.max_patches);
      }
      return ASD_OK;
    };
    if ((rc = build()) != ASD_OK) {
      for (auto& S : ax->slots) slot_free(S);
      for (hipEvent_t e : ax->ev_corners) if (e) (void)hipEventDestroy(e);
      for (hipStream_t st : ax->stream_f) if (st) { (void)hipStreamDestroy(st); }
      for (int w = 1; w < kWorkers; ++w) fe_free(ax->fe[w]);
      if (sx) { (void)hipStreamDestroy(sx); }
      delete ax;
      return rc;
    }
    ctx->stream_x = sx;
    ctx->ax = ax;
    static const int n_workers = [] { const char* e = getenv("ASD_EXTRACT_WORKERS"); const int v = e ? atoi(e) : kWorkers; return v < 1 ? 1 : (v > kWorkers ? kWorkers : v); }();
    for (int w = 0; w < n_workers; ++w) ax->th[w] = std::thread(async_worker, ctx, w);
  }
  AsyncExtract* ax = ctx->ax;
  if (ctx->adopt_pending) {
    ASD_HIP_CHECK(ctx, hipStreamWaitEvent(ctx->stream_x, ctx->ev_adopt, 0));
    ctx->adopt_pending = false;
  }
  {
    std::lock_guard<std::mutex> l(ax->m);
    if (ax->submitted - ax->waited >= (uint64_t)kQueueDepth) {
      ctx->set_error("asd_extract_submit: %d submissions are already outstanding", kQueueDepth);
      return ASD_ERR_CAPACITY;
    }
    AsyncJob& a = ax->jobs[ax->submitted % kSlots];
    a.job = ExtractJob();
    a.job.image = image; a.job.on_device = device_resident != 0; a.job.w = width; a.job.h = height; a.job.stride = stride;
    a.job.nfeat = n_features_override;
    a.state = AsyncJob::QUEUED;
    ++ax->submitted;
  }
  ax->cv.notify_all();
  return ASD_OK;
}

static AsyncJob* wait_oldest(asd_ctx* ctx, int* rc) {
  AsyncExtract* ax = ctx->ax;
  AsyncJob* a;
  bool back;
  {
    std::unique_lock<std::mutex> l(ax->m);
    if (ax->waited == ax->submitted) { ctx->set_error("asd_extract_wait: nothing was submitted"); *rc = ASD_ERR_INVALID; return nullptr; }
    a = &ax->jobs[ax->waited % kSlots];
    if (ax->hold_back && a->state != AsyncJob::BACK && a->state != AsyncJob::DONE) { ax->hold_back = false; ax->cv.notify_all(); }
    ax->cv.wait(l, [&] { return a->state == AsyncJob::BACK || a->state == AsyncJob::DONE; });
    back = a->state == AsyncJob::BACK;
  }
  if (back) {
    (void)hipSetDevice(ctx->cfg.device);
    const int frc = extract_finish(ctx, ax->slots[a->slot], a->job.n, a->kps.data(), nullptr);
    std::lock_guard<std::mutex> l(ax->m);
    if (frc != ASD_OK) a->job.rc = frc;
    a->state = AsyncJob::DONE;
  }
  {
    std::lock_guard<std::mutex> l(ax->m);
    ++ax->waited;
    if (a->job.rc == ASD_OK) ax->last_view = ax->waited - 1;
  }
  if (a->job.rc != ASD_OK) { *rc = a->job.rc; return nullptr; }
  ctx->last_n = a->job.n;
  ctx->d_desc_last = ax->slots[a->slot].d_desc;
  ctx->d_pyr_view = ctx->keep_pyramid ? ax->slots[a->slot].d_pyr_keep : nullptr;
  *rc = ASD_OK;
  return a;
}

int asd_extract_wait(asd_ctx* ctx, asd_keypoint* kps, float* desc, int32_t* n_out) {
  if (!ctx || !ctx->ax || !kps || !desc || !n_out) return ASD_ERR_INVALID;
  int rc;
  AsyncJob* a = wait_oldest(ctx, &rc);
  if (!a) return rc;
  const int n = a->job.n;
  memcpy(kps, a->kps.data(), (size_t)n * sizeof(asd_keypoint));
  memcpy(desc, ctx->ax->slots[a->slot].h_desc, (size_t)n * 128 * sizeof(float));
  *n_out = n;
  return ASD_OK;
}

int asd_extract_wait_view(asd_ctx* ctx, const asd_keypoint** kps, const float** desc, int32_t* n_out) {
  if (!ctx || !ctx->ax || !kps || !desc || !n_out) return ASD_ERR_INVALID;
  int rc;
  AsyncJob* a = wait_oldest(ctx, &rc);
  if (!a) return rc;
  *kps = a->kps.data();
  *desc = ctx->ax->slots[a->slot].h_desc;
  *n_out = a->job.n;
  return ASD_OK;
}

uint64_t asd_extract_last_view(const asd_ctx* ctx) {
  if (!ctx || !ctx->ax) return ~0ull;
  std::lock_guard<std::mutex> l(ctx->ax->m);
  return ctx->ax->last_view;
}

int32_t asd_extract_view_valid(asd_ctx* ctx, uint64_t view_id) {
  if (!ctx || !ctx->ax) return 0;
  AsyncExtract* ax = ctx->ax;
  std::lock_guard<std::mutex> l(ax->m);
  return view_id < ax->waited && ax->submitted <= view_id + (uint64_t)kSlots ? 1 : 0;
}

int asd_get_level_size(const asd_ctx* ctx, int32_t level, int32_t* width, int32_t* height) {
  if (!ctx || !ctx->fe || !width || !height || level < 0 || level >= ctx->fe->pyr.nlevels) return ASD_ERR_INVALID;
  *width = ctx->fe->pyr.lv[level].w;
  *height = ctx->fe->pyr.lv[level].h;
  return ASD_OK;
}

int asd_get_level_image(asd_ctx* ctx, int32_t level, int32_t blurred, uint8_t* out) {
  if (!ctx || !ctx->fe || !out || level < 0 || level >= ctx->fe->pyr.nlevels) return ASD_ERR_INVALID;
  if (asd_extractor_busy(ctx, "asd_get_level_image")) return ASD_ERR_INVALID;
  const LevelDev& L = ctx->fe->pyr.lv[level];
  const uint8_t* src = (blurred ? ctx->fe->d_blur : ctx->fe->d_pyr) + L.off;
  ASD_HIP_CHECK(ctx, hipMemcpy2DAsync(out, L.w, src, L.pitch, L.w, L.h, hipMemcpyDeviceToHost, ctx->stream));
  ASD_HIP_CHECK(ctx, hipStreamSynchronize(ctx->stream));
  return ASD_OK;
}

int asd_get_raw_corners(asd_ctx* ctx, int32_t level, int32_t capacity, float* x, float* y, float* response, int32_t* n_out) {
  if (!ctx || !ctx->fe || !n_out || level < 0 || level >= ctx->fe->pyr.nlevels) return ASD_ERR_INVALID;
  if (asd_extractor_busy(ctx, "asd_get_raw_corners")) return ASD_ERR_INVALID;
  const FrontendState* fe = ctx->fe;
  const int n = std::min((int)fe->raw_x[level].size(), capacity);
  for (int i = 0; i < n; ++i) {
    if (x) x[i] = fe->raw_x[level][i];
    if (y) y[i] = fe->raw_y[level][i];
    if (response) response[i] = fe->raw_r[level][i];
  }
  *n_out = n;
  return ASD_OK;
}

int asd_get_patches(asd_ctx* ctx, int32_t capacity, uint8_t* out, int32_t* n_out) {
  if (!ctx || !ctx->fe || !n_out || capacity < 0 || (capacity > 0 && !out)) return ASD_ERR_INVALID;
  if (asd_extractor_busy(ctx, "asd_get_patches")) return ASD_ERR_INVALID;
  const int n = std::min(ctx->patches_n, (int)capacity);
  if (n > 0) {
    ASD_HIP_CHECK(ctx, hipMemcpyAsync(out, ctx->d_patches, (size_t)n * 1024, hipMemcpyDeviceToHost, ctx->stream));
    ASD_HIP_CHECK(ctx, hipStreamSynchronize(ctx->stream));
  }
  *n_out = n;
  return ASD_OK;
}

}

namespace {

struct StereoArgs {
  PyrDev P;
  const uint8_t *pyr_l, *pyr_r;
  const float4 *kp_l, *kp_r;
  const float *desc_l, *desc_r;
  const int *row_start, *row_items;
  int n_l, n_rows;
  float maxD, mbf;
  float scale[ASD_MAX_LEVELS], inv_scale[ASD_MAX_LEVELS];
  float* u_right; float* depth; int* sad;
};

__global__ __launch_bounds__(256) void k_stereo_match(StereoArgs a) {
  const int lane = threadIdx.x & 63;
  const int iL = blockIdx.x * 4 + (threadIdx.x >> 6);
  if (iL >= a.n_l) return;
  const float4 kl = a.kp_l[iL];
  const float uL = kl.x, vL = kl.y;
  const int levelL = __float_as_int(kl.z);
  float out_u = -1.0f, out_d = -1.0f;
  int out_sad = -1;
  const int row = (int)vL;
  do {
    if (row < 0 || row >= a.n_rows) break;
    const int c0 = a.row_start[row], c1 = a.row_start[row + 1];
    if (c0 == c1) break;
    const float minU = uL - a.maxD, maxU = uL;
    if (maxU < 0) break;
    float best = 1.5f;
    int best_pos = 0x7fffffff;
    const float4* dl = reinterpret_cast<const float4*>(a.desc_l + (size_t)iL * 128);
    for (int p = c0 + lane; p < c1; p += 64) {
      const int iR = a.row_items[p];
      const float4 kr = a.kp_r[iR];
      const int oR = __float_as_int(kr.z);
      if (oR < levelL - 1 || oR > levelL + 1) continue;
      if (!(kr.x >= minU && kr.x <= maxU)) continue;
      const float4* dr = reinterpret_cast<const float4*>(a.desc_r + (size_t)iR * 128);
      float acc = 0.f;
      for (int k = 0; k < 32; ++k) {
        const float4 x = dl[k], y = dr[k];
        float d;
        d = x.x - y.x; acc = acc + d * d;
        d = x.y - y.y; acc = acc + d * d;
        d = x.z - y.z; acc = acc + d * d;
        d = x.w - y.w; acc = acc + d * d;
      }
      if (acc < best) { best = acc; best_pos = p; }
    }
    for (int off = 32; off >= 1; off >>= 1) {
      const float ob = __shfl_xor(best, off);
      const int op = __shfl_xor(best_pos, off);
      if (ob < best || (ob == best && op < best_pos)) { best = ob; best_pos = op; }
    }
    if (!(best < 1.0f) || best_pos == 0x7fffffff) break;
    const int iR = a.row_items[best_pos];
    const float uR0 = a.kp_r[iR].x;
    const float sf = a.inv_scale[levelL];
    const float scaleduL = roundf(uL * sf), scaledvL = roundf(vL * sf), scaleduR0 = roundf(uR0 * sf);
    const LevelDev Lv = a.P.lv[levelL];
    const float iniu = scaleduR0 + 5 - 5, endu = scaleduR0 + 5 + 5 + 1;
    if (iniu < 0 || endu >= Lv.w) break;
    const int xl = (int)scaleduL, yl = (int)scaledvL, xr = (int)scaleduR0;
    if (xl - 5 < 0 || xl + 5 >= Lv.w || yl - 5 < 0 || yl + 5 >= Lv.h || xr - 10 < 0 || xr + 10 >= Lv.w) break;
    const uint8_t* L0 = a.pyr_l + Lv.off;
    const uint8_t* R0 = a.pyr_r + Lv.off;
    const int cl = L0[yl * Lv.pitch + xl];
    int sad[11];
#pragma unroll
    for (int s = 0; s < 11; ++s) sad[s] = 0;
    for (int q = lane; q < 121; q += 64) {
      const int dy = q / 11 - 5, dx = q % 11 - 5;
      const int il = (int)L0[(yl + dy) * Lv.pitch + xl + dx] - cl;
      const uint8_t* rrow = R0 + (yl + dy) * Lv.pitch + xr + dx;
#pragma unroll
      for (int s = 0; s < 11; ++s) {
        const int cr = R0[yl * Lv.pitch + xr + (s - 5)];
        const int ir = (int)rrow[s - 5] - cr;
        sad[s] += abs(il - ir);
      }
    }
#pragma unroll
    for (int s = 0; s < 11; ++s)
      for (int off = 32; off >= 1; off >>= 1) sad[s] += __shfl_xor(sad[s], off);
    float bestS = 2147483648.0f;
    int bestinc = 0;
    float vd[11];
#pragma unroll
    for (int s = 0; s < 11; ++s) {
      vd[s] = (float)sad[s];
      if (vd[s] < bestS) { bestS = vd[s]; bestinc = s - 5; }
    }
    if (bestinc == -5 || bestinc == 5) break;
    float d1 = 0.f, d2 = 0.f, d3 = 0.f;
#pragma unroll
    for (int s = 1; s < 10; ++s)
      if (s - 5 == bestinc) { d1 = vd[s - 1]; d2 = vd[s]; d3 = vd[s + 1]; }
    const float deltaR = (d1 - d3) / (2.0f * (d1 + d3 - 2.0f * d2));
    if (deltaR < -1 || deltaR > 1) break;
    float bestuR = a.scale[levelL] * ((float)scaleduR0 + (float)bestinc + deltaR);
    float disparity = uL - bestuR;
    if (disparity >= 0.f && disparity < a.maxD) {
      if (disparity <= 0) { disparity = 0.01; bestuR = uL - 0.01; }
      out_d = a.mbf / disparity;
      out_u = bestuR;
      out_sad = (int)bestS;
    }
  } while (false);
  if (lane == 0) { a.u_right[iL] = out_u; a.depth[iL] = out_d; a.sad[iL] = out_sad; }
}

}

extern "C" int asd_stereo_match(asd_ctx* ctx_left, asd_ctx* ctx_right, int32_t slot_left, int32_t slot_right, float mb, float mbf,
                                float* u_right, float* depth, int32_t* n_matched) {
  if (!ctx_left || !ctx_right || !u_right || !depth || !n_matched || slot_left < 0 || slot_left >= ASD_MAX_FRAMES || slot_right < 0 ||
      slot_right >= ASD_MAX_FRAMES || !(mb > 0) || !(mbf > 0))
    return ASD_ERR_INVALID;
  asd_ctx* ctx = ctx_left;
  if (ctx_left->cfg.device != ctx_right->cfg.device) { ctx->set_error("asd_stereo_match: both contexts must live on the same device"); return ASD_ERR_INVALID; }
  FrontendState *fl = ctx_left->fe, *fr = ctx_right->fe;
  if (fl && fl->cfg_w == 0 && ctx_left->ax && ctx_left->ax->fe[1]) fl = ctx_left->ax->fe[1];
  if (fr && fr->cfg_w == 0 && ctx_right->ax && ctx_right->ax->fe[1]) fr = ctx_right->ax->fe[1];
  if (!fl || !fr || fl->cfg_w == 0 || fl->cfg_w != fr->cfg_w || fl->cfg_h != fr->cfg_h) {
    ctx->set_error("asd_stereo_match: extract the left and the right image (same size) on the two contexts first");
    return ASD_ERR_INVALID;
  }
  const AsdFrameSlot &FL = ctx->frames[slot_left], &FR = ctx->frames[slot_right];
  const int N = FL.n, Nr = FR.n;
  *n_matched = 0;
  for (int i = 0; i < N; ++i) { u_right[i] = -1.0f; depth[i] = -1.0f; }
  if (!FL.d_kp || !FR.d_kp) { ctx->set_error("asd_stereo_match: frame slot not set"); return ASD_ERR_INVALID; }
  if (N == 0 || Nr == 0) return ASD_OK;
  const bool views = ctx_left->d_pyr_view && ctx_right->d_pyr_view;
  if (!views) {
// ... 75 lines not shown
```

asd-slam_amd/host/asd_adapters.hpp:

```cpp
#pragma once
#include <cstdint>
#include <stdexcept>
#include <string>
#include <utility>
#include <algorithm>
#include <vector>

#include "../../include/asd_slam.h"

namespace asd {

struct Camera { float fx, fy, cx, cy; };

struct FrameView {
  int slot = 0;
  std::vector<asd_keypoint> mvKeysUn;
  std::vector<float> mDescriptors;
  float mnMinX = 0, mnMaxX = 0, mnMinY = 0, mnMaxY = 0;
  float mTcw[16] = {1, 0, 0, 0, 0, 1, 0, 0, 0, 0, 1, 0, 0, 0, 0, 1};
  std::vector<int32_t> mvpMapPoints;
  std::vector<uint8_t> mvbOutlier;
  int N() const { return (int)mvKeysUn.size(); }
};

struct MapPointView {
  float Xw[3];
  float normal[3];
  float mfMinDistance, mfMaxDistance;
  const float* descriptor;
  int nObs = 1;
};

class Context {
 public:
  Context(int nfeatures, float scaleFactor, int nlevels, int iniThFAST, int minThFAST, int maxWidth, int maxHeight,
          int device = 0) {
    asd_config cfg{nfeatures, scaleFactor, nlevels, iniThFAST, minThFAST, maxWidth, maxHeight, 2 * nfeatures, device};
    const int rc = asd_ctx_create(&cfg, &ctx_);
    if (rc != ASD_OK) throw std::runtime_error("asd_ctx_create failed (" + std::to_string(rc) + "): no usable HIP device");
  }
  ~Context() { if (ctx_) asd_ctx_destroy(ctx_); }
  Context(const Context&) = delete;
  Context& operator=(const Context&) = delete;
  asd_ctx* get() const { return ctx_; }
  const char* error() const { return asd_last_error(ctx_); }
  void SetUndistortion(const float K[4], const float distCoef[4], int width, int height) {
    if (asd_set_undistortion(ctx_, K, distCoef, width, height) != ASD_OK) throw std::runtime_error(error());
  }
 private:
  asd_ctx* ctx_ = nullptr;
};

class ORBextractor {
 public:
  ORBextractor(Context& c, const float* const conv_w[7], const float* const bn_mean[7], const float* const bn_var[7],
               float bn_eps = 1e-5f)
      : c_(c) {
    if (asd_load_weights(c_.get(), conv_w, bn_mean, bn_var, bn_eps) != ASD_OK) throw std::runtime_error(c_.error());
    asd_config dummy{};
    (void)dummy;
  }
  int ExtractDesc(const uint8_t* image, int width, int height, int stride, std::vector<asd_keypoint>& keypoints,
                  std::vector<float>& descriptors, int nfeatures_override = 0) {
    const int cap = capacity();
    keypoints.resize(cap);
    descriptors.resize((size_t)cap * ASD_DESC_DIM);
    int32_t n = 0;
    if (asd_extract(c_.get(), image, width, height, stride, nfeatures_override, keypoints.data(), descriptors.data(), &n) != ASD_OK)
      return -1;
    keypoints.resize(n);
    descriptors.resize((size_t)n * ASD_DESC_DIM);
    return n;
  }
  int GetLevels() const { return levels(); }
  std::vector<float> GetScaleFactors() const { return table(0); }
  std::vector<float> GetInverseScaleFactors() const { return table(1); }
  std::vector<float> GetScaleSigmaSquares() const { return table(2); }
  std::vector<float> GetInverseScaleSigmaSquares() const { return table(3); }
  std::vector<uint8_t> ImagePyramidLevel(int level, int* w, int* h) const {
    int32_t ww = 0, hh = 0;
    if (asd_get_level_size(c_.get(), level, &ww, &hh) != ASD_OK) return {};
    std::vector<uint8_t> img((size_t)ww * hh);
    asd_get_level_image(c_.get(), level, 0, img.data());
    *w = ww; *h = hh;
    return img;
  }
 private:
  int levels() const { int n = 0; float s[ASD_MAX_LEVELS]; int32_t f[ASD_MAX_LEVELS]; asd_get_scale_tables(c_.get(), s, nullptr, nullptr, nullptr, f); for (; n < ASD_MAX_LEVELS && f[n] > 0; ++n) {} return n; }
  int capacity() const { return 1 << 13; }
  std::vector<float> table(int which) const {
    float t[4][ASD_MAX_LEVELS] = {};
    asd_get_scale_tables(c_.get(), t[0], t[1], t[2], t[3], nullptr);
    return std::vector<float>(t[which], t[which] + levels());
  }
  Context& c_;
};

inline int FrameAssignFeaturesToGrid(Context& c, FrameView& F, bool adopt_last_extract = true) {
  return asd_frame_set(c.get(), F.slot, F.mvKeysUn.data(), adopt_last_extract ? nullptr : F.mDescriptors.data(), F.N(),
                       F.mnMinX, F.mnMaxX, F.mnMinY, F.mnMaxY);
}

class ORBmatcher {
 public:
  ORBmatcher(Context& c, float nnratio = 0.6f, bool checkOri = true) : c_(c), mfNNratio(nnratio), mbCheckOrientation(checkOri) {}

  float DescriptorDistance(const float* a, const float* b) {
    float d = -1.f;
    asd_dist_matrix(c_.get(), a, 1, b, 1, &d);
    return d;
  }

  int SearchByProjection(FrameView& Cur, const FrameView& Last, const std::vector<const MapPointView*>& points,
                         const Camera& K, float th, bool  = true) {
    const int nl = Last.N();
    std::vector<uint8_t> has(nl, 0), obs(nl, 1);
    std::vector<float> Xw((size_t)nl * 3, 0.f), desc((size_t)nl * ASD_DESC_DIM, 0.f);
    for (int i = 0; i < nl; ++i)
      if (points[i]) {
        has[i] = 1;
        obs[i] = points[i]->nObs > 0;
        for (int k = 0; k < 3; ++k) Xw[3 * i + k] = points[i]->Xw[k];
        for (int k = 0; k < ASD_DESC_DIM; ++k) desc[(size_t)i * ASD_DESC_DIM + k] = points[i]->descriptor[k];
      }
    std::vector<int32_t> match(Cur.N(), -1);
    int32_t n = 0;
    const float Kv[4] = {K.fx, K.fy, K.cx, K.cy};
    if (asd_match_project_frame(c_.get(), Cur.slot, Last.slot, has.data(), Xw.data(), desc.data(), Cur.mTcw, Kv, th,
                                mbCheckOrientation, match.data(), &n, obs.data()) != ASD_OK)
      return 0;
    Cur.mvpMapPoints.assign(Cur.N(), -1);
    for (int j = 0; j < Cur.N(); ++j)
      if (match[j] >= 0) Cur.mvpMapPoints[j] = Last.mvpMapPoints[match[j]];
    return n;
  }

  int SearchByProjection(FrameView& F, const std::vector<MapPointView>& vpMapPoints, const std::vector<int32_t>& ids,
                         const Camera& K, float th = 3.f) {
    const int n = (int)vpMapPoints.size();
    std::vector<float> Xw((size_t)n * 3), nrm((size_t)n * 3), mind(n), maxd(n), desc((size_t)n * ASD_DESC_DIM);
    for (int m = 0; m < n; ++m) {
      for (int k = 0; k < 3; ++k) { Xw[3 * m + k] = vpMapPoints[m].Xw[k]; nrm[3 * m + k] = vpMapPoints[m].normal[k]; }
      mind[m] = vpMapPoints[m].mfMinDistance; maxd[m] = vpMapPoints[m].mfMaxDistance;
      for (int k = 0; k < ASD_DESC_DIM; ++k) desc[(size_t)m * ASD_DESC_DIM + k] = vpMapPoints[m].descriptor[k];
    }
    std::vector<uint8_t> in_view(n), occupied(F.N(), 0), obs(n, 1);
    for (int m = 0; m < n; ++m) obs[m] = vpMapPoints[m].nObs > 0;
    std::vector<float> proj((size_t)n * 2), vc(n);
    std::vector<int32_t> level(n), match(F.N(), -1);
    const float Kv[4] = {K.fx, K.fy, K.cx, K.cy};
    if (asd_frustum(c_.get(), F.slot, n, Xw.data(), nrm.data(), mind.data(), maxd.data(), F.mTcw, Kv, 0.5f,
                    in_view.data(), proj.data(), level.data(), vc.data()) != ASD_OK)
      return 0;
    for (int j = 0; j < F.N(); ++j) occupied[j] = F.mvpMapPoints.size() == (size_t)F.N() && F.mvpMapPoints[j] >= 0;
    int32_t nm = 0;
    if (asd_match_project_points(c_.get(), F.slot, n, in_view.data(), proj.data(), level.data(), vc.data(), desc.data(),
                                 occupied.data(), th, mfNNratio, match.data(), &nm, obs.data()) != ASD_OK)
      return 0;
    F.mvpMapPoints.resize(F.N(), -1);
    for (int j = 0; j < F.N(); ++j)
      if (match[j] >= 0) F.mvpMapPoints[j] = ids[match[j]];
    return nm;
  }

  int SearchForInitialization(const FrameView& F1, const FrameView& F2, std::vector<float>& vbPrevMatched,
                              std::vector<int>& vnMatches12, int windowSize = 10) {
    vnMatches12.assign(F1.N(), -1);
    int32_t n = 0;
    if (asd_match_init(c_.get(), F1.slot, F2.slot, vbPrevMatched.data(), windowSize, mfNNratio, mbCheckOrientation,
                       vnMatches12.data(), &n) != ASD_OK)
      return 0;
    return n;
  }

  struct FeatVec {
    std::vector<int32_t> node, start{0}, idx;
    asd_feature_vector view() const { return asd_feature_vector{(int32_t)node.size(), node.data(), start.data(), idx.data()}; }
  };

  int SearchByBoW(const FrameView& KF, const FeatVec& fvKF, const FrameView& F, const FeatVec& fvF,
                  std::vector<int32_t>& vpMapPointMatches) {
    std::vector<uint8_t> has(KF.N(), 0);
    for (int i = 0; i < KF.N(); ++i) has[i] = KF.mvpMapPoints.size() == (size_t)KF.N() && KF.mvpMapPoints[i] >= 0;
    std::vector<int32_t> m(F.N(), -1);
    int32_t n = 0;
    const asd_feature_vector a = fvKF.view(), b = fvF.view();
    if (asd_match_bow(c_.get(), KF.slot, F.slot, &a, &b, has.data(), mfNNratio, mbCheckOrientation, m.data(), &n) != ASD_OK) return 0;
    vpMapPointMatches.assign(F.N(), -1);
    for (int j = 0; j < F.N(); ++j)
      if (m[j] >= 0) vpMapPointMatches[j] = KF.mvpMapPoints[m[j]];
    return n;
  }

  int SearchByBoW(const FrameView& KF1, const FeatVec& fv1, const FrameView& KF2, const FeatVec& fv2, std::vector<int32_t>& vpMatches12,
                  std::vector<int32_t>& vnIdx2) {
    std::vector<uint8_t> h1(KF1.N(), 0), h2(KF2.N(), 0);
    for (int i = 0; i < KF1.N(); ++i) h1[i] = KF1.mvpMapPoints.size() == (size_t)KF1.N() && KF1.mvpMapPoints[i] >= 0;
    for (int i = 0; i < KF2.N(); ++i) h2[i] = KF2.mvpMapPoints.size() == (size_t)KF2.N() && KF2.mvpMapPoints[i] >= 0;
    vnIdx2.assign(KF1.N(), -1);
    vpMatches12.assign(KF1.N(), -1);
    int32_t n = 0;
    const asd_feature_vector a = fv1.view(), b = fv2.view();
    if (asd_match_bow_kf(c_.get(), KF1.slot, KF2.slot, &a, &b, h1.data(), h2.data(), mfNNratio, mbCheckOrientation, vnIdx2.data(), &n) != ASD_OK) {
      vnIdx2.assign(KF1.N(), -1);
      return 0;
    }
    for (int i = 0; i < KF1.N(); ++i)
      if (vnIdx2[i] >= 0) vpMatches12[i] = KF2.mvpMapPoints[vnIdx2[i]];
    return n;
  }

  int SearchForTriangulation(const FrameView& KF1, const FeatVec& fv1, const FrameView& KF2, const FeatVec& fv2, const float F12[9],
                             float ex, float ey, std::vector<std::pair<size_t, size_t>>& vMatchedPairs) {
    std::vector<uint8_t> h1(KF1.N(), 0), h2(KF2.N(), 0);
    for (int i = 0; i < KF1.N(); ++i) h1[i] = KF1.mvpMapPoints.size() == (size_t)KF1.N() && KF1.mvpMapPoints[i] >= 0;
    for (int i = 0; i < KF2.N(); ++i) h2[i] = KF2.mvpMapPoints.size() == (size_t)KF2.N() && KF2.mvpMapPoints[i] >= 0;
    std::vector<int32_t> m(KF1.N(), -1);
    int32_t n = 0;
    const asd_feature_vector a = fv1.view(), b = fv2.view();
    vMatchedPairs.clear();
    if (asd_match_triangulate(c_.get(), KF1.slot, KF2.slot, &a, &b, h1.data(), h2.data(), F12, ex, ey, mbCheckOrientation, m.data(), &n) != ASD_OK)
      return 0;
    for (int i = 0; i < KF1.N(); ++i)
      if (m[i] >= 0) vMatchedPairs.emplace_back((size_t)i, (size_t)m[i]);
    return n;
  }

  int Fuse(const FrameView& KF, const std::vector<MapPointView>& vpMapPoints, const std::vector<uint8_t>& valid, const Camera& K,
           std::vector<int32_t>& bestIdx, float th = 3.f) {
    const int n = (int)vpMapPoints.size();
    std::vector<float> Xw((size_t)n * 3), nrm((size_t)n * 3), mind(n), maxd(n), desc((size_t)n * ASD_DESC_DIM), bd(n);
    for (int m = 0; m < n; ++m) {
      for (int k = 0; k < 3; ++k) { Xw[3 * m + k] = vpMapPoints[m].Xw[k]; nrm[3 * m + k] = vpMapPoints[m].normal[k]; }
      mind[m] = vpMapPoints[m].mfMinDistance; maxd[m] = vpMapPoints[m].mfMaxDistance;
      for (int k = 0; k < ASD_DESC_DIM; ++k) desc[(size_t)m * ASD_DESC_DIM + k] = vpMapPoints[m].descriptor[k];
    }
    bestIdx.assign(n, -1);
    const float Kv[4] = {K.fx, K.fy, K.cx, K.cy};
    if (asd_fuse_search(c_.get(), KF.slot, n, valid.data(), Xw.data(), nrm.data(), mind.data(), maxd.data(), desc.data(), KF.mTcw, Kv, th,
                        bestIdx.data(), bd.data()) != ASD_OK)
      return 0;
    int nFused = 0;
    for (int m = 0; m < n; ++m) nFused += bestIdx[m] >= 0;
    return nFused;
  }

 private:
  Context& c_;
  float mfNNratio;
  bool mbCheckOrientation;
};

struct Optimizer {
// ... 350 lines not shown
```

asd-slam_amd/host/track_loop.cpp:

```cpp
#include <algorithm>
#include <cmath>
#include <cstdint>
#include <cstdio>
#include <chrono>
#include <cstdlib>
#include <cstring>
#include <deque>
#include <vector>

#include "track_loop.h"

extern "C" {

struct asd_track_handle {
  asd_ctx* ctx;
  std::vector<const uint8_t*> d_frames;
  int W, H;
  float K32[4], T[16], scale32[8];
  double K64[4], pose0[7], inv_sigma2[8];
  asd_ba_problem ba;
  int kf_interval, lookahead;
  bool fused = true;
  bool async_ba = false;
  bool split = true;
  bool chain = false;
  int tables_for = -1;
  int map_copies = 2;
  const asd_do_mapping_inputs* dm = nullptr;
  std::vector<int32_t> dm_matches, dm_nmatch, dm_best, dm_distinct;
  std::vector<float> dm_x3d, dm_bdist;
  std::vector<uint8_t> dm_ok;
  double dm_ms = 0.0;
  long dm_calls = 0;
  asd_ctx* ctx_r = nullptr;
  std::vector<const uint8_t*> d_frames_r;
  float mb = 0.f, mbf = 0.f;
  std::vector<float> u_right, depth_r;
  std::vector<asd_keypoint> kps_r;
  std::vector<float> desc_sync_r;
  int32_t prep_stereo = -1;
  int frames_on_host = 0;
  int bank_base = 0;
  std::vector<int32_t> last_cand, cand_rows, sel_rows;
  asd_track_frame_args fa;
  int32_t f_n1 = 0, f_inl1 = 0, f_n2 = 0, f_inl2 = 0;
  double f_pose[7], f_pose1[7];
  float drift_cx = 620.5f, drift_cy = 188.0f, drift_z = 1.003f, drift_dx = 3.0f, drift_dy = 0.2f;
  int stop_after = -1;
  int prep_t = -1;
  const asd_keypoint* prep_kps = nullptr;
  int32_t prep_n = 0;
  int32_t c2_n2 = 0, c2_ninl = 0;
  double c2_pose[7];
  std::vector<uint8_t> outl2;
  bool ba_out = false;
  long ba_step = -1;
  asd_ba_problem ba_p;
  asd_ba_result ba_r;
  int slot = 0;
  std::deque<int> pending;
  bool have_last = false;
  std::vector<asd_keypoint> last_kps;
  int last_slot = 0;
  std::vector<asd_keypoint> kps;
  std::vector<float> desc_sync;
  std::vector<float> uv, Xw, Xw2, nrm, dist, maxd, mind, proj, vc;
  std::vector<uint8_t> has, in_view, occ, outl;
  std::vector<float> cur_Xw, Xs, ns, mind_s, maxd_s;
  std::vector<int32_t> sel;
  std::vector<uint8_t> keep, in_frame;
  std::vector<double> ba_obs;
  float T1[16];
  std::vector<int32_t> rows, m1, m2, level;
  std::vector<double> Xd, obs, info;
  std::vector<double> ba_poses, ba_points, ba_chi2;
  std::vector<uint8_t> ba_dpos, ba_out1;
  double wait_ms = 0.0, ba_ms = 0.0;
  double ba_prep_ms = 0.0;
  double seg_ms[8] = {};
  double kern_ms[4] = {};
  long steps = 0;
};

asd_track_handle* asd_track_create(asd_ctx* ctx, int32_t n_frames, const void* const* d_frames, int32_t W, int32_t H, const float* K32,
                                   const float* T, const double* pose0, const double* inv_sigma2, const float* scale32,
                                   const asd_ba_problem* ba, int32_t kf_interval, int32_t lookahead) {
  if (!ctx || n_frames < 1 || !d_frames || !K32 || !T || !pose0 || !inv_sigma2 || !scale32 || !ba || kf_interval < 1 || lookahead < 0 ||
      lookahead > ASD_EXTRACT_QUEUE)
    return nullptr;
  asd_track_handle* h = new asd_track_handle();
  h->ctx = ctx;
  for (int i = 0; i < n_frames; ++i) h->d_frames.push_back(static_cast<const uint8_t*>(d_frames[i]));
  h->W = W; h->H = H;
  for (int i = 0; i < 4; ++i) { h->K32[i] = K32[i]; h->K64[i] = (double)K32[i]; }
  memcpy(h->T, T, sizeof h->T);
  memcpy(h->pose0, pose0, sizeof h->pose0);
  memcpy(h->inv_sigma2, inv_sigma2, sizeof h->inv_sigma2);
  memcpy(h->scale32, scale32, sizeof h->scale32);
  h->ba = *ba;
  h->kf_interval = kf_interval; h->lookahead = lookahead;
  h->kps.resize(1 << 13);
  h->desc_sync.resize((size_t)(1 << 13) * 128);
  return h;
}

void asd_track_set_fused(asd_track_handle* h, int32_t on) { if (h) h->fused = on != 0; }
void asd_track_set_async_ba(asd_track_handle* h, int32_t on) { if (h) h->async_ba = on != 0; }
void asd_track_set_split(asd_track_handle* h, int32_t on) { if (h) h->split = on != 0; }
void asd_track_set_chain(asd_track_handle* h, int32_t on) { if (h) h->chain = on != 0; }
void asd_track_set_map_copies(asd_track_handle* h, int32_t copies) { if (h && copies >= 1 && copies <= 16) h->map_copies = copies; }
int asd_track_drain(asd_track_handle* h) {
  if (!h) return ASD_ERR_INVALID;
  int rc = ASD_OK;
  while (!h->pending.empty()) {
    const asd_keypoint* k; const float* d; int32_t n;
    const int r = asd_extract_wait_view(h->ctx, &k, &d, &n);
    if (r != ASD_OK) rc = r;
    if (h->ctx_r) { const int r2 = asd_extract_wait_view(h->ctx_r, &k, &d, &n); if (r2 != ASD_OK) rc = r2; }
    h->pending.pop_front();
  }
  h->prep_t = -1;
  h->have_last = false;
  return rc;
}
void asd_track_set_frames_on_host(asd_track_handle* h, int32_t on) { if (h) h->frames_on_host = on != 0; }
int asd_track_set_stereo(asd_track_handle* h, asd_ctx* ctx_right, const void* const* d_frames_right, float mb, float mbf) {
  if (!h || !ctx_right || !d_frames_right || !(mb > 0) || !(mbf > 0) || !h->pending.empty()) return ASD_ERR_INVALID;
  int rc;
  if ((rc = asd_extract_keep_pyramid(h->ctx, 1)) != ASD_OK || (rc = asd_extract_keep_pyramid(ctx_right, 1)) != ASD_OK) return rc;
  h->ctx_r = ctx_right;
  h->d_frames_r.clear();
  for (size_t i = 0; i < h->d_frames.size(); ++i) h->d_frames_r.push_back(static_cast<const uint8_t*>(d_frames_right[i]));
  h->mb = mb; h->mbf = mbf;
  return ASD_OK;
}
void asd_track_set_do_mapping(asd_track_handle* h, const asd_do_mapping_inputs* in, int32_t n_cur) {
  if (!h) return;
  h->dm = in;
  if (!in) return;
  h->dm_matches.assign((size_t)in->n_nb * n_cur, -1); h->dm_nmatch.assign(std::max(in->n_nb, 1), 0);
  h->dm_x3d.assign((size_t)in->n_nb * n_cur * 3, 0.f); h->dm_ok.assign((size_t)in->n_nb * n_cur, 0);
  h->dm_best.assign(std::max(in->n_fuse_total, 1), -1); h->dm_bdist.assign(std::max(in->n_fuse_total, 1), 0.f);
  h->dm_distinct.assign(std::max(in->n_sets, 1), 0);
}
void asd_track_get_do_mapping_times(const asd_track_handle* h, double* ms, int64_t* calls) {
  if (!h) return;
  if (ms) *ms = h->dm_ms;
  if (calls) *calls = h->dm_calls;
}
void asd_track_get_times(const asd_track_handle* h, double* ba_ms, double* extract_wait_ms, int64_t* steps) {
  if (!h) return;
  if (ba_ms) *ba_ms = h->ba_ms;
  if (extract_wait_ms) *extract_wait_ms = h->wait_ms;
  if (steps) *steps = h->steps;
}
void asd_track_set_drift(asd_track_handle* h, float cx, float cy, float z, float dx, float dy) {
  if (h) { h->drift_cx = cx; h->drift_cy = cy; h->drift_z = z; h->drift_dx = dx; h->drift_dy = dy; }
}

static int collect_ba(asd_track_handle* h, asd_track_stats* st, long st_step) {
  if (!h->ba_out) return ASD_OK;
  const auto b0 = std::chrono::steady_clock::now();
  const int rc = asd_local_ba_wait(h->ctx);
  h->ba_ms += std::chrono::duration<double, std::milli>(std::chrono::steady_clock::now() - b0).count();
  h->ba_out = false;
  if (rc != ASD_OK) return rc;
  if (st && st_step == h->ba_step) { st->ba_chi2 = h->ba_r.chi2_second; st->has_ba = 1; }
  return ASD_OK;
}

void asd_track_destroy(asd_track_handle* h) {
  if (!h) return;
  while (!h->pending.empty()) {
    const asd_keypoint* k; const float* d; int32_t n;
    (void)asd_extract_wait_view(h->ctx, &k, &d, &n);
    if (h->ctx_r) (void)asd_extract_wait_view(h->ctx_r, &k, &d, &n);
    h->pending.pop_front();
  }
  (void)collect_ba(h, nullptr, -1);
  if (getenv("ASD_TIMING") && h->steps)
  {
    fprintf(stderr, "[track_loop] steps %ld  extract wait %.3f ms/step  local BA %.3f ms/step (+ %.3f ms/step putting its problem together on the host)\n", h->steps,
            h->wait_ms / h->steps, h->ba_ms / h->steps, h->ba_prep_ms / h->steps);
    static const char* nm[8] = {"frame_set", "submit", "bank+M1", "pose1", "frustum", "M2", "pose2", "host glue"};
    for (int i = 0; i < 8; ++i) fprintf(stderr, "[track_loop]   %-10s %.3f ms/step\n", nm[i], h->seg_ms[i] / h->steps);
    fprintf(stderr, "[track_loop]   device time: M1 %.3f pose1 %.3f M2 %.3f pose2 %.3f ms/step\n", h->kern_ms[0] / h->steps, h->kern_ms[1] / h->steps,
            h->kern_ms[2] / h->steps, h->kern_ms[3] / h->steps);
  }
  delete h;
}

static void build_candidate_tables(asd_track_handle* h, int nl) {
  const std::vector<asd_keypoint>& lk = h->last_kps;
  const int nc = h->map_copies * nl;
  h->Xw2.resize((size_t)3 * nc); h->nrm.resize((size_t)3 * nc); h->dist.resize(nc); h->maxd.resize(nc); h->mind.resize(nc);
  for (int c = 0; c < h->map_copies; ++c)
    for (int i = 0; i < nl; ++i)
      for (int k = 0; k < 3; ++k) h->Xw2[3 * ((size_t)c * nl + i) + k] = c == 0 ? h->Xw[3 * i + k] : h->Xw[3 * i + k] + (c == 1 ? 0.02f : 0.02f * (float)c);
  for (int i = 0; i < nc; ++i) {
    const float* P = &h->Xw2[3 * (size_t)i];
    const float nn = std::sqrt((P[0] * P[0] + P[1] * P[1]) + P[2] * P[2]);
    for (int k = 0; k < 3; ++k) h->nrm[3 * (size_t)i + k] = P[k] / nn;
    h->dist[i] = nn;
    const int lv = lk[i % nl].octave;
    h->maxd[i] = nn * h->scale32[lv];
    h->mind[i] = h->maxd[i] / h->scale32[7];
  }
}

static int prepare_frame(asd_track_handle* h, int t, const std::vector<int>& next) {
  asd_ctx* ctx = h->ctx;
  asd_ctx* ctxr = h->ctx_r;
  const int nf = (int)h->d_frames.size();
  int rc;
  auto tp = std::chrono::steady_clock::now();
  auto seg = [&](int i) {
    const auto now = std::chrono::steady_clock::now();
    h->seg_ms[i] += std::chrono::duration<double, std::milli>(now - tp).count();
    tp = now;
  };
  auto drop_pending = [&]() -> int {
    while (!h->pending.empty()) {
      const asd_keypoint* k; const float* d; int32_t nn;
      int r = asd_extract_wait_view(ctx, &k, &d, &nn);
      if (r == ASD_OK && ctxr) r = asd_extract_wait_view(ctxr, &k, &d, &nn);
      if (r != ASD_OK) return r;
      h->pending.pop_front();
    }
    return ASD_OK;
  };
  const asd_keypoint *kps = nullptr, *kps_r = nullptr;
  int32_t n = 0, n_r = 0;
  if (!h->pending.empty() && h->pending.front() == t) {
    const float* d = nullptr;
    const auto w0 = std::chrono::steady_clock::now();
    if ((rc = asd_extract_wait_view(ctx, &kps, &d, &n)) != ASD_OK) return rc;
    if (ctxr && (rc = asd_extract_wait_view(ctxr, &kps_r, &d, &n_r)) != ASD_OK) return rc;
    h->wait_ms += std::chrono::duration<double, std::milli>(std::chrono::steady_clock::now() - w0).count();
    h->pending.pop_front();
  } else {
    if ((rc = drop_pending()) != ASD_OK) return rc;
    if ((rc = (h->frames_on_host ? asd_extract : asd_extract_device)(ctx, h->d_frames[t % nf], h->W, h->H, h->W, 0, h->kps.data(), h->desc_sync.data(), &n)) != ASD_OK) return rc;
    kps = h->kps.data();
    if (ctxr) {
      h->kps_r.resize(1 << 13); h->desc_sync_r.resize((size_t)(1 << 13) * 128);
      if ((rc = asd_extract_device(ctxr, h->d_frames_r[t % nf], h->W, h->H, h->W, 0, h->kps_r.data(), h->desc_sync_r.data(), &n_r)) != ASD_OK) return rc;
      kps_r = h->kps_r.data();
    }
  }
  const bool chain = h->fused && h->split;
  if (chain) h->slot = (h->slot + 1) % 3; else h->slot ^= 1;
  seg(7);
  if ((rc = asd_frame_set(ctx, h->slot, kps, nullptr, n, 0.f, (float)h->W, 0.f, (float)h->H)) != ASD_OK) return rc;
  seg(0);
  if (ctxr) {
    const int slot_r = 3 + h->slot;
    if ((rc = asd_frame_set_from_ctx(ctx, slot_r, kps_r, n_r, 0.f, (float)h->W, 0.f, (float)h->H, ctxr)) != ASD_OK) return rc;
    h->u_right.resize(std::max(n, 1)); h->depth_r.resize(std::max(n, 1));
    int32_t nm = 0;
    if ((rc = asd_stereo_match(ctx, ctxr, h->slot, slot_r, h->mb, h->mbf, h->u_right.data(), h->depth_r.data(), &nm)) != ASD_OK) return rc;
    h->prep_stereo = nm;
    seg(4);
  }
  if (h->lookahead > 0) {
    bool same = h->pending.size() <= next.size();
    for (size_t i = 0; same && i < h->pending.size(); ++i) same = h->pending[i] == next[i];
    if (!same && (rc = drop_pending()) != ASD_OK) return rc;
    for (size_t i = h->pending.size(); i < next.size(); ++i) {
      if ((rc = asd_extract_submit(ctx, h->d_frames[next[i] % nf], h->frames_on_host ? 0 : 1, h->W, h->H, h->W, 0)) != ASD_OK) return rc;
      if (ctxr && (rc = asd_extract_submit(ctxr, h->d_frames_r[next[i] % nf], 1, h->W, h->H, h->W, 0)) != ASD_OK) return rc;
      h->pending.push_back(next[i]);
    }
  }
  seg(1);
  if (h->have_last && chain) {
    const std::vector<asd_keypoint>& lk = h->last_kps;
    const int nl = (int)lk.size();
    const float fx = h->K32[0], fy = h->K32[1], cx = h->K32[2], cy = h->K32[3];
    const float z = h->drift_z, c3 = (float)((double)h->drift_dx * (double)(h->drift_z == 1.003f ? 1.003 : (double)h->drift_z)),
                c02 = (float)((double)(h->drift_dy == 0.2f ? 0.2 : (double)h->drift_dy) * (double)(h->drift_z == 1.003f ? 1.003 : (double)h->drift_z)), depth = 20.0f;
    h->Xw.resize((size_t)3 * nl);
    for (int i = 0; i < nl; ++i) {
      const float u = (lk[i].x - h->drift_cx) * z + h->drift_cx - c3;
      const float v = (lk[i].y - h->drift_cy) * z + h->drift_cy - c02;
      h->Xw[3 * i + 0] = (u - cx) / fx * depth;
      h->Xw[3 * i + 1] = (v - cy) / fy * depth;
      h->Xw[3 * i + 2] = depth;
    }
    const int n2p = h->map_copies * nl;
    build_candidate_tables(h, nl);
    seg(7);
    h->bank_base = h->bank_base ? 0 : 65536;
    const int base = h->bank_base;
    if (n2p > 65536) return ASD_ERR_CAPACITY;
    for (int c = 0; c < h->map_copies; ++c)
      if ((rc = asd_bank_put_from_frame(ctx, h->last_slot, base + c * nl, nl)) != ASD_OK) return rc;
    if ((rc = asd_mpbank_put(ctx, base, n2p, h->Xw2.data(), h->nrm.data(), h->mind.data(), h->maxd.data())) != ASD_OK) return rc;
    h->rows.resize(nl); h->last_cand.resize(nl); h->cand_rows.resize(n2p);
    for (int i = 0; i < nl; ++i) { h->rows[i] = base + i; h->last_cand[i] = i; }
    for (int i = 0; i < n2p; ++i) h->cand_rows[i] = base + i;
    h->tables_for = t;
    seg(2);
  } else if (h->have_last) {
    const std::vector<asd_keypoint>& lk = h->last_kps;
    const int nl = (int)lk.size();
    const float fx = h->K32[0], fy = h->K32[1], cx = h->K32[2], cy = h->K32[3];
    const float z = h->drift_z, c3 = (float)((double)h->drift_dx * (double)(h->drift_z == 1.003f ? 1.003 : (double)h->drift_z)),
                c02 = (float)((double)(h->drift_dy == 0.2f ? 0.2 : (double)h->drift_dy) * (double)(h->drift_z == 1.003f ? 1.003 : (double)h->drift_z)), depth = 20.0f;
    h->Xw.resize((size_t)3 * nl);
    for (int i = 0; i < nl; ++i) {
      const float u = (lk[i].x - h->drift_cx) * z + h->drift_cx - c3;
      const float v = (lk[i].y - h->drift_cy) * z + h->drift_cy - c02;
      h->Xw[3 * i + 0] = (u - cx) / fx * depth;
      h->Xw[3 * i + 1] = (v - cy) / fy * depth;
      h->Xw[3 * i + 2] = depth;
    }
    seg(7);
    for (int c = 0; c < h->map_copies; ++c)
      if ((rc = asd_bank_put_from_frame(ctx, h->last_slot, c * nl, nl)) != ASD_OK) return rc;
    h->rows.resize((size_t)h->map_copies * nl);
    for (int i = 0; i < h->map_copies * nl; ++i) h->rows[i] = i;
    build_candidate_tables(h, nl);
    if ((rc = asd_mpbank_put(ctx, 0, h->map_copies * nl, h->Xw2.data(), h->nrm.data(), h->mind.data(), h->maxd.data())) != ASD_OK) return rc;
    h->tables_for = t;
    seg(2);
  }
  h->prep_t = t; h->prep_kps = kps; h->prep_n = n;
  return ASD_OK;
}

static int submit_ba(asd_track_handle* h, asd_track_stats* st, int t);

// ... 451 lines not shown
```

include/asd_slam.h:

```cpp
#ifndef ASD_SLAM_H
#define ASD_SLAM_H

#include <stdint.h>

#ifdef __cplusplus
extern "C" {
#endif

#define ASD_DESC_DIM 128
#define ASD_PATCH 32
#define ASD_MAX_LEVELS 16
#define ASD_GRID_COLS 64
#define ASD_GRID_ROWS 48
#define ASD_HISTO_LENGTH 30

typedef enum asd_status {
  ASD_OK = 0,
  ASD_ERR_INVALID = -1,
  ASD_ERR_NO_DEVICE = -2,
  ASD_ERR_HIP = -3,
  ASD_ERR_NO_WEIGHTS = -4,
  ASD_ERR_CAPACITY = -5,
  ASD_ERR_NUMERIC = -6,
  ASD_ERR_RANGE = -7
} asd_status;

typedef struct asd_ctx asd_ctx;

typedef struct asd_config {
  int32_t n_features;
  float   scale_factor;
  int32_t n_levels;
  int32_t ini_th_fast;
  int32_t min_th_fast;
  int32_t max_width;
  int32_t max_height;
  int32_t max_patches;
  int32_t device;
} asd_config;

typedef struct asd_keypoint {
  float   x, y;
  float   size;
  float   angle;
  float   response;
  int32_t octave;
} asd_keypoint;

int asd_ctx_create(const asd_config* cfg, asd_ctx** out);
int asd_ctx_destroy(asd_ctx* ctx);
const char* asd_last_error(const asd_ctx* ctx);
const char* asd_version(void);

int asd_get_scale_tables(const asd_ctx* ctx, float* scale, float* inv_scale, float* sigma2,
                         float* inv_sigma2, int32_t* features_per_level);

int asd_load_weights(asd_ctx* ctx, const float* const conv_w[7], const float* const bn_mean[7],
                     const float* const bn_var[7], float bn_eps);

int asd_describe(asd_ctx* ctx, const uint8_t* patches, int32_t n, float* desc);

int asd_describe_device(asd_ctx* ctx, const uint8_t* d_patches, int32_t n, float* d_desc);

int asd_extract(asd_ctx* ctx, const uint8_t* image, int32_t width, int32_t height, int32_t stride,
                int32_t n_features_override, asd_keypoint* kps, float* desc, int32_t* n_out);

int asd_extract_device(asd_ctx* ctx, const uint8_t* d_image, int32_t width, int32_t height, int32_t stride,
                       int32_t n_features_override, asd_keypoint* kps, float* desc, int32_t* n_out);

#define ASD_EXTRACT_QUEUE 3
int asd_extract_submit(asd_ctx* ctx, const uint8_t* image, int32_t device_resident, int32_t width,
                       int32_t height, int32_t stride, int32_t n_features_override);
int asd_extract_wait(asd_ctx* ctx, asd_keypoint* kps, float* desc, int32_t* n_out);
int asd_extract_wait_view(asd_ctx* ctx, const asd_keypoint** kps, const float** desc, int32_t* n_out);
uint64_t asd_extract_last_view(const asd_ctx* ctx);
int32_t asd_extract_view_valid(asd_ctx* ctx, uint64_t view_id);

int asd_get_level_size(const asd_ctx* ctx, int32_t level, int32_t* width, int32_t* height);
int asd_get_level_image(asd_ctx* ctx, int32_t level, int32_t blurred, uint8_t* out);
int asd_get_raw_corners(asd_ctx* ctx, int32_t level, int32_t capacity, float* x, float* y,
                        float* response, int32_t* n_out);
int asd_get_patches(asd_ctx* ctx, int32_t capacity, uint8_t* out, int32_t* n_out);

int asd_undistort_map(const float K[4], const float dist[4], int32_t width, int32_t height, int16_t* xy, uint16_t* frac);
int asd_set_undistortion(asd_ctx* ctx, const float K[4], const float dist[4], int32_t width, int32_t height);
int asd_undistort(asd_ctx* ctx, const uint8_t* src, int32_t device_resident, int32_t width, int32_t height, int32_t stride,
                  uint8_t* dst, int32_t dst_stride);

#define ASD_MAX_FRAMES 64
int asd_frame_set(asd_ctx* ctx, int32_t slot, const asd_keypoint* kps, const float* desc,
                  int32_t n, float min_x, float max_x, float min_y, float max_y);

int asd_frame_features_in_area(asd_ctx* ctx, int32_t slot, float x, float y, float r,
                               int32_t min_level, int32_t max_level, int32_t capacity,
                               int32_t* idx_out, int32_t* n_out);

int asd_dist_matrix(asd_ctx* ctx, const float* a, int32_t na, const float* b, int32_t nb, float* out);

int asd_distinctive_descriptor(asd_ctx* ctx, const float* desc, int32_t n, int32_t* best_idx);
int asd_distinctive_descriptor_batch(asd_ctx* ctx, int32_t n_sets, const int32_t* set_start, const float* desc,
                                     int32_t* best_idx);

int asd_match_project_frame(asd_ctx* ctx, int32_t slot_cur, int32_t slot_last,
                            const uint8_t* has_mp, const float* Xw, const float* mp_desc,
                            const float* Tcw, const float* K, float th, int32_t check_orientation,
                            int32_t* match_cur, int32_t* n_matches, const uint8_t* mp_obs_positive);

int asd_match_project_points(asd_ctx* ctx, int32_t slot_cur, int32_t n_mp, const uint8_t* in_view,
                             const float* proj, const int32_t* level, const float* view_cos,
                             const float* desc, const uint8_t* occupied, float th, float nn_ratio,
                             int32_t* match_cur, int32_t* n_matches, const uint8_t* mp_obs_positive);

int asd_bank_put(asd_ctx* ctx, int32_t first_row, int32_t n, const float* desc);
int asd_bank_put_from_frame(asd_ctx* ctx, int32_t slot, int32_t first_row, int32_t n);
int asd_match_project_frame_bank(asd_ctx* ctx, int32_t slot_cur, int32_t slot_last,
                                 const uint8_t* has_mp, const float* Xw, const int32_t* mp_rows,
                                 const float* Tcw, const float* K, float th, int32_t check_orientation,
                                 int32_t* match_cur, int32_t* n_matches, const uint8_t* mp_obs_positive);
int asd_match_project_points_bank(asd_ctx* ctx, int32_t slot_cur, int32_t n_mp, const uint8_t* in_view,
                                  const float* proj, const int32_t* level, const float* view_cos,
                                  const int32_t* rows, const uint8_t* occupied, float th, float nn_ratio,
                                  int32_t* match_cur, int32_t* n_matches, const uint8_t* mp_obs_positive);

int asd_track_motion_model(asd_ctx* ctx, int32_t slot_cur, int32_t slot_last, const uint8_t* has_mp, const float* Xw,
                           const float* mp_desc, const float* Tcw, const float* K, float th, int32_t check_orientation,
                           const uint8_t* mp_obs_positive, double* pose7, int32_t* match_cur, int32_t* n_matches,
                           uint8_t* outlier, int32_t* n_inliers);
int asd_track_motion_model_bank(asd_ctx* ctx, int32_t slot_cur, int32_t slot_last, const uint8_t* has_mp, const float* Xw,
                                const int32_t* mp_rows, const float* Tcw, const float* K, float th, int32_t check_orientation,
                                const uint8_t* mp_obs_positive, double* pose7, int32_t* match_cur, int32_t* n_matches,
                                uint8_t* outlier, int32_t* n_inliers);
int asd_track_local_map(asd_ctx* ctx, int32_t slot_cur, int32_t n_mp, const uint8_t* in_view, const float* proj,
                        const int32_t* level, const float* view_cos, const float* desc, const float* mp_Xw,
                        const uint8_t* occupied, const float* cur_Xw, float th, float nn_ratio,
                        const uint8_t* mp_obs_positive, const float* K, double* pose7, int32_t* match_cur,
                        int32_t* n_matches, uint8_t* outlier, int32_t* n_inliers);
int asd_track_local_map_bank(asd_ctx* ctx, int32_t slot_cur, int32_t n_mp, const uint8_t* in_view, const float* proj,
                             const int32_t* level, const float* view_cos, const int32_t* rows, const float* mp_Xw,
                             const uint8_t* occupied, const float* cur_Xw, float th, float nn_ratio,
                             const uint8_t* mp_obs_positive, const float* K, double* pose7, int32_t* match_cur,
                             int32_t* n_matches, uint8_t* outlier, int32_t* n_inliers);

int asd_track_local_points(asd_ctx* ctx, int32_t slot_cur, int32_t n_mp, const float* Xw, const float* normal,
                           const float* min_dist, const float* max_dist, const float* desc, const float* Tcw, const float* K,
                           float viewing_cos_limit, const uint8_t* occupied, const float* cur_Xw, float th, float nn_ratio,
                           const uint8_t* mp_obs_positive, double* pose7, int32_t* match_cur, int32_t* n_matches,
                           uint8_t* outlier, int32_t* n_inliers);
int asd_track_local_points_bank(asd_ctx* ctx, int32_t slot_cur, int32_t n_mp, const float* Xw, const float* normal,
                                const float* min_dist, const float* max_dist, const int32_t* rows, const float* Tcw,
                                const float* K, float viewing_cos_limit, const uint8_t* occupied, const float* cur_Xw, float th,
                                float nn_ratio, const uint8_t* mp_obs_positive, double* pose7, int32_t* match_cur,
                                int32_t* n_matches, uint8_t* outlier, int32_t* n_inliers);

int asd_track_local_points_rows(asd_ctx* ctx, int32_t slot_cur, int32_t n_mp, const int32_t* rows, const float* Tcw, const float* K,
                                float viewing_cos_limit, const uint8_t* occupied, const float* cur_Xw, float th, float nn_ratio,
                                const uint8_t* mp_obs_positive, double* pose7, int32_t* match_cur, int32_t* n_matches, uint8_t* outlier,
                                int32_t* n_inliers);

int asd_mpbank_put(asd_ctx* ctx, int32_t first_row, int32_t n, const float* Xw, const float* normal, const float* min_dist,
                   const float* max_dist);

typedef struct asd_track_frame_args {
  int32_t slot_cur, slot_last;
  const uint8_t* has_mp;
  const float* Xw_last;
  const int32_t* last_rows;
  const int32_t* last_cand;
  const uint8_t* last_obs_positive;
  const float* Tcw;
  float th;
  int32_t check_orientation;
  int32_t n_cand;
  const int32_t* cand_rows;
  const uint8_t* cand_obs_positive;
  float viewing_cos_limit, th_local, nn_ratio;
  const float* K;
  double* pose7;
  double* pose1;
  int32_t *match1, *n_matches1; uint8_t* outlier1; int32_t* n_inliers1;
  int32_t *match2, *n_matches2; uint8_t* outlier2; int32_t* n_inliers2;
} asd_track_frame_args;
int asd_track_frame(asd_ctx* ctx, const asd_track_frame_args* args);

int asd_prep_async(asd_ctx* ctx, int32_t on);

int asd_track_async(asd_ctx* ctx);
int asd_track_finish(asd_ctx* ctx);

int asd_frustum(asd_ctx* ctx, int32_t slot_cur, int32_t n, const float* Xw, const float* normal,
                const float* min_dist, const float* max_dist, const float* Tcw, const float* K,
                float viewing_cos_limit, uint8_t* in_view, float* proj, int32_t* level, float* view_cos);

int asd_match_init(asd_ctx* ctx, int32_t slot1, int32_t slot2, float* prev_matched, int32_t window,
                   float nn_ratio, int32_t check_orientation, int32_t* matches12, int32_t* n_matches);

typedef struct asd_feature_vector {
  int32_t n_nodes;
  const int32_t* node_id;
  const int32_t* start;
  const int32_t* idx;
} asd_feature_vector;


int asd_match_project_keyframe(asd_ctx* ctx, int32_t slot_cur, int32_t n_kf, const uint8_t* valid, const float* Xw,
                               const float* min_dist, const float* max_dist, const float* desc, const float* kf_angle,
                               const uint8_t* occupied, const float* Tcw, const float* K, float th, float orb_dist,
                               int32_t check_orientation, int32_t* match_cur, int32_t* n_matches);

int asd_match_project_sim3(asd_ctx* ctx, int32_t slot_kf, const float* Scw, int32_t n_mp, const uint8_t* valid,
                           const float* Xw, const float* normal, const float* min_dist, const float* max_dist,
                           const float* desc, const float* K, int32_t th, int32_t* matched_kp, int32_t* n_matches);

int asd_fuse_search_sim3(asd_ctx* ctx, int32_t slot_kf, const float* Scw, int32_t n_mp, const uint8_t* valid,
                         const float* Xw, const float* normal, const float* min_dist, const float* max_dist,
                         const float* desc, const float* K, float th, int32_t* best_idx, float* best_dist);

int asd_match_sim3(asd_ctx* ctx, int32_t slot1, int32_t slot2, const uint8_t* has1, const uint8_t* has2, const float* Xw1,
                   const float* Xw2, const float* min_dist1, const float* max_dist1, const float* min_dist2,
                   const float* max_dist2, const float* desc1, const float* desc2, const float* T1w, const float* T2w,
                   float s12, const float* R12, const float* t12, const float* K, float th, int32_t* match12,
                   int32_t* n_matches);

int asd_voc_load(asd_ctx* ctx, int32_t n_nodes, int32_t k, int32_t L, int32_t weighting, int32_t scoring,
                 const int32_t* child_start, const int32_t* child_ids, const double* weight,
                 const int32_t* word_id, const float* desc);
int asd_bow_descend(asd_ctx* ctx, int32_t slot, const float* desc, int32_t n, int32_t levelsup, int32_t* word,
                    int32_t* node, double* weight);
// ... 142 lines not shown
```

Baseline: 1256.

## Skip per-frame descriptor download in track loop and fuse patch stats into angle kernel

The tracking loop now turns off the automatic device-to-host copy of descriptors after each extraction, since tracking uses the device-resident descriptors, and adds an on-demand fetch API for callers that still need them on the host. Separately, the per-patch mean/std normalisation stats are computed inside the angle/patch kernel with wave reductions and passed to the network, removing a separate k_patch_stats launch. This saves a 2000x128 float copy per frame and one kernel launch. In exchange, host consumers must fetch explicitly, and the angle kernel does extra reduction work.

```diff
diff --git a/asd-slam_amd/capi.py b/asd-slam_amd/capi.py
--- a/asd-slam_amd/capi.py
+++ b/asd-slam_amd/capi.py
@@ -248,16 +248,39 @@
             pk, pd = C.c_void_p(), C.c_void_p()
             self._chk(self.lib.asd_extract_wait_view(self.ctx, C.byref(pk), C.byref(pd), C.byref(n)))
             if n.value == 0:
-                return np.zeros(0, KP_DTYPE), np.zeros((0, 128), np.float32)
+                return np.zeros(0, KP_DTYPE), (np.zeros((0, 128), np.float32) if pd.value else None)
             kb = (C.c_char * (n.value * KP_DTYPE.itemsize)).from_address(pk.value)
+            kps = np.frombuffer(kb, dtype=KP_DTYPE, count=n.value)
+            if not pd.value:
+                return kps, None
             db = (C.c_float * (n.value * 128)).from_address(pd.value)
-            return np.frombuffer(kb, dtype=KP_DTYPE, count=n.value), np.frombuffer(db, dtype=np.float32).reshape(n.value, 128)
+            return kps, np.frombuffer(db, dtype=np.float32).reshape(n.value, 128)
         cap = self.cfg.max_patches
         if not hasattr(self, "_kps_buf"):
             self._kps_buf = np.zeros(cap, KP_DTYPE)
             self._desc_buf = np.empty((cap, 128), np.float32)
         self._chk(self.lib.asd_extract_wait(self.ctx, _p(self._kps_buf), _p(self._desc_buf), C.byref(n)))
         return self._kps_buf[:n.value], self._desc_buf[:n.value]
+
+    def extract_host_descriptors(self, on=True):
+        self._chk(self.lib.asd_extract_host_descriptors(self.ctx, int(on)))
+
+    def extract_host_descriptors_enabled(self):
+        self.lib.asd_extract_host_descriptors_enabled.restype = C.c_int32
+        return bool(self.lib.asd_extract_host_descriptors_enabled(self.ctx))
+
+    def extract_fetch_descriptors(self, n):
+        out = np.empty((n, 128), np.float32)
+        self._chk(self.lib.asd_extract_fetch_descriptors(self.ctx, _p(out)))
+        return out
+
+    def debug_front_stats(self):
+        cap = self.cfg.max_patches
+        front, ref = np.empty((cap, 2), np.float32), np.empty((cap, 2), np.float32)
+        n = C.c_int32()
+        self.lib.asd_debug_front_stats.argtypes = [C.c_void_p, C.c_int32, C.c_void_p, C.c_void_p, C.c_void_p]
+        self._chk(self.lib.asd_debug_front_stats(self.ctx, cap, _p(front), _p(ref), C.byref(n)))
+        return front[:n.value].copy(), ref[:n.value].copy()
 
     def extract_last_view(self):
         self.lib.asd_extract_last_view.restype = C.c_uint64
diff --git a/asd-slam_amd/csrc/asdnet.hip b/asd-slam_amd/csrc/asdnet.hip
--- a/asd-slam_amd/csrc/asdnet.hip
+++ b/asd-slam_amd/csrc/asdnet.hip
@@ -1356,16 +1356,22 @@
 
 int asdnet_profile_collect_set(asd_ctx* ctx, int set);
 
-static int asdnet_forward_one(asd_ctx* ctx, const uint8_t* d_patches, int n, float* d_desc, hipStream_t st, int* range_flag);
-int asdnet_forward_device(asd_ctx* ctx, const uint8_t* d_patches, int n, float* d_desc, hipStream_t st, int* range_flag) {
+static int asdnet_forward_one(asd_ctx* ctx, const uint8_t* d_patches, int n, float* d_desc, hipStream_t st, int* range_flag, const float* d_stats);
+int asdnet_patch_stats(asd_ctx* ctx, const uint8_t* d_patches, int n, float* d_stats, hipStream_t st) {
+  if (n <= 0) return ASD_OK;
+  hipLaunchKernelGGL(k_patch_stats, dim3(n), dim3(256), 0, st, d_patches, d_stats, n);
+  ASD_HIP_CHECK(ctx, hipGetLastError());
+  return ASD_OK;
+}
+int asdnet_forward_device(asd_ctx* ctx, const uint8_t* d_patches, int n, float* d_desc, hipStream_t st, int* range_flag, const float* d_stats) {
   if (!ctx->weights_loaded) { ctx->set_error("asd_load_weights has not been called"); return ASD_ERR_NO_WEIGHTS; }
   if (n < 0 || n > ctx->cfg.max_patches) { ctx->set_error("n=%d exceeds max_patches=%d", n, ctx->cfg.max_patches); return ASD_ERR_CAPACITY; }
   if (n == 0) return ASD_OK;
   if (!st) st = ctx->stream;
   std::lock_guard<std::mutex> prof_lock(ctx->prof_mutex);
-  return asdnet_forward_one(ctx, d_patches, n, d_desc, st, range_flag);
-}
-static int asdnet_forward_one(asd_ctx* ctx, const uint8_t* d_patches, int n, float* d_desc, hipStream_t st, int* range_flag) {
+  return asdnet_forward_one(ctx, d_patches, n, d_desc, st, range_flag, d_stats);
+}
+static int asdnet_forward_one(asd_ctx* ctx, const uint8_t* d_patches, int n, float* d_desc, hipStream_t st, int* range_flag, const float* d_stats) {
   float *a0 = ctx->d_act[0], *a1 = ctx->d_act[1];
   const int npad = (n + 31) / 32 * 32;
   const bool prof = ctx->prof_on;
@@ -1387,9 +1393,13 @@
                                      1.f / (kActScale * ctx->wx2_scale[l]), x3_stats)                                                               \
       : launch_conv_x3<CFG, FUSE, 3>(st, src, ctx->d_wx3[l], ctx->d_bias[l], dst, n, w1p, b1p, nullptr, nullptr, 1.f, 1.f,                \
                                      x3_stats))
-    hipLaunchKernelGGL(k_patch_stats, dim3(n), dim3(256), 0, st, d_patches, ctx->d_part, n);
-    ASD_HIP_CHECK(ctx, hipGetLastError());
-    x3_stats = ctx->d_part;
+    if (d_stats && !ctx->d_calib) {
+      x3_stats = d_stats;
+    } else {
+      hipLaunchKernelGGL(k_patch_stats, dim3(n), dim3(256), 0, st, d_patches, ctx->d_part, n);
+      ASD_HIP_CHECK(ctx, hipGetLastError());
+      x3_stats = ctx->d_part;
+    }
     ASD_HIP_CHECK(ctx, (X3_LAUNCH(L2S_CFG, true, 1, d_patches, a1, ctx->d_w1, ctx->d_bias[0])));
     x3_stats = nullptr;
     CALIB(1, a1, 32 * 32 * 32);
diff --git a/asd-slam_amd/csrc/ctx.h b/asd-slam_amd/csrc/ctx.h
--- a/asd-slam_amd/csrc/ctx.h
+++ b/asd-slam_amd/csrc/ctx.h
@@ -258,6 +258,9 @@
   const uint8_t* d_pyr_view = nullptr;
   AsdDevBuf stereo_scratch;
   float* d_desc_last = nullptr;
+  float* h_desc_last = nullptr;
+  uint64_t desc_last_view = ~0ull;
+  bool host_desc = true;
   hipEvent_t ev_adopt = nullptr;
   bool adopt_pending = false;
 
@@ -355,5 +358,7 @@
 void asdnet_free(asd_ctx* ctx);
 int asdnet_load_weights(asd_ctx* ctx, const float* const conv_w[7], const float* const bn_mean[7],
                         const float* const bn_var[7], float eps);
-int asdnet_forward_device(asd_ctx* ctx, const uint8_t* d_patches, int n, float* d_desc, hipStream_t st, int* range_flag = nullptr);
+int asdnet_forward_device(asd_ctx* ctx, const uint8_t* d_patches, int n, float* d_desc, hipStream_t st, int* range_flag = nullptr,
+                          const float* d_stats = nullptr);
+int asdnet_patch_stats(asd_ctx* ctx, const uint8_t* d_patches, int n, float* d_stats, hipStream_t st);
 int asdnet_profile_collect(asd_ctx* ctx);
diff --git a/asd-slam_amd/csrc/frontend.hip b/asd-slam_amd/csrc/frontend.hip
--- a/asd-slam_amd/csrc/frontend.hip
+++ b/asd-slam_amd/csrc/frontend.hip
@@ -275,7 +275,8 @@
 
 __global__ __launch_bounds__(256) void k_angle_patch(PyrDev P, const uint8_t* __restrict__ pyr,
                                                      const uint8_t* __restrict__ blur, const short4* __restrict__ kps,
-                                                     int n, float* __restrict__ angles, uint8_t* __restrict__ patches) {
+                                                     int n, float* __restrict__ angles, uint8_t* __restrict__ patches,
+                                                     float* __restrict__ stats) {
   const int lane = threadIdx.x & 63;
   const int k = blockIdx.x * 4 + (threadIdx.x >> 6);
   if (k >= n) return;
@@ -301,6 +302,41 @@
     w[q] = (uint32_t)src[q * 4] | ((uint32_t)src[q * 4 + 1] << 8) | ((uint32_t)src[q * 4 + 2] << 16) |
            ((uint32_t)src[q * 4 + 3] << 24);
   *reinterpret_cast<uint4*>(patches + (size_t)k * 1024 + row * 32 + half * 16) = make_uint4(w[0], w[1], w[2], w[3]);
+  const float inv255 = (float)(1.0 / 255);
+  float x[16];
+#pragma unroll
+  for (int i = 0; i < 16; ++i) {
+    x[i] = (float)((w[i >> 2] >> (8 * (i & 3))) & 255u) * inv255;
+    asm volatile("" : "+v"(x[i]));
+  }
+  float s[4];
+#pragma unroll
+  for (int j = 0; j < 4; ++j) s[j] = (x[4 * j] + x[4 * j + 1]) + (x[4 * j + 2] + x[4 * j + 3]);
+#pragma unroll
+  for (int off = 8; off >= 1; off >>= 1)
+#pragma unroll
+    for (int j = 0; j < 4; ++j) s[j] += __shfl_xor(s[j], off);
+  float sum = (s[0] + s[2]) + (s[1] + s[3]);
+  sum += __shfl_xor(sum, 16);
+  sum += __shfl_xor(sum, 32);
+  const float mean = sum * (1.0f / 1024.0f);
+#pragma unroll
+  for (int j = 0; j < 4; ++j) {
+    const float d0 = x[4 * j] - mean, d1 = x[4 * j + 1] - mean, d2 = x[4 * j + 2] - mean, d3 = x[4 * j + 3] - mean;
+    float q = d1 * d1;
+    q = __builtin_fmaf(d0, d0, q);
+    q = __builtin_fmaf(d2, d2, q);
+    s[j] = __builtin_fmaf(d3, d3, q);
+  }
+#pragma unroll
+  for (int off = 8; off >= 1; off >>= 1)
+#pragma unroll
+    for (int j = 0; j < 4; ++j) s[j] += __shfl_xor(s[j], off);
+  float ss = (s[0] + s[2]) + (s[1] + s[3]);
+  ss += __shfl_xor(ss, 16);
+  ss += __shfl_xor(ss, 32);
+  const float sd = sqrtf(ss * (1.0f / 1023.0f)) + 1e-7f;
+  if (lane == 0) *reinterpret_cast<float2*>(stats + 2 * (size_t)k) = make_float2(mean, sd);
 }
 
 
@@ -363,6 +399,7 @@
   uint8_t* d_patches = nullptr;
   float* d_desc = nullptr;
   float *d_angles = nullptr, *h_angles = nullptr, *h_desc = nullptr;
+  float* d_stats = nullptr;
   int* h_range = nullptr;
   hipEvent_t ev_begin = nullptr, ev_front = nullptr, ev_end = nullptr;
   bool owned = false;
@@ -388,6 +425,7 @@
   int* h_level_start = nullptr;
   short4 *d_kps = nullptr, *h_kps = nullptr;
   float *d_angles = nullptr, *h_angles = nullptr, *h_desc = nullptr;
+  float* d_stats = nullptr;
   std::vector<float> raw_x[ASD_MAX_LEVELS], raw_y[ASD_MAX_LEVELS], raw_r[ASD_MAX_LEVELS];
   std::vector<int> sel[ASD_MAX_LEVELS];
   LevelPool* pool = nullptr;
@@ -442,6 +480,7 @@
   ASD_HIP_CHECK(ctx, hipMalloc(&fe->d_angles, np * sizeof(float)));
   ASD_HIP_CHECK(ctx, hipHostMalloc(&fe->h_angles, (np + 16) * sizeof(float)));
   ASD_HIP_CHECK(ctx, hipHostMalloc(&fe->h_desc, np * 128 * sizeof(float)));
+  ASD_HIP_CHECK(ctx, hipMalloc(&fe->d_stats, np * 2 * sizeof(float)));
   return ASD_OK;
 }
 int frontend_alloc(asd_ctx* ctx) { return fe_alloc(ctx, &ctx->fe); }
@@ -450,7 +489,7 @@
   if (!fe) return;
   void* dev[] = {fe->d_pyr, fe->d_blur, fe->d_score, fe->d_xofs, fe->d_ialpha, fe->d_yofs, fe->d_ibeta, fe->d_cells,
                  fe->d_cell_count, fe->d_cell_off, fe->d_level_cell_start, fe->d_level_start,
-                 fe->d_kps, fe->d_angles, fe->d_stage};
+                 fe->d_kps, fe->d_angles, fe->d_stage, fe->d_stats};
   for (void* p : dev) if (p) (void)hipFree(p);
   void* host[] = {fe->h_corners, fe->h_level_start, fe->h_kps, fe->h_angles, fe->h_desc};
   for (void* p : host) if (p) (void)hipHostFree(p);
@@ -587,6 +626,7 @@
   ASD_HIP_CHECK(ctx, hipMalloc(&S.d_patches, np * 1024));
   ASD_HIP_CHECK(ctx, hipMalloc(&S.d_desc, np * 128 * sizeof(float)));
   ASD_HIP_CHECK(ctx, hipMalloc(&S.d_angles, np * sizeof(float)));
+  ASD_HIP_CHECK(ctx, hipMalloc(&S.d_stats, np * 2 * sizeof(float)));
   ASD_HIP_CHECK(ctx, hipHostMalloc(&S.h_angles, (np + 16) * sizeof(float)));
   S.h_range = reinterpret_cast<int*>(S.h_angles + np);
   ASD_HIP_CHECK(ctx, hipHostMalloc(&S.h_desc, np * 128 * sizeof(float)));
@@ -604,6 +644,7 @@
     if (S.d_patches) (void)hipFree(S.d_patches);
     if (S.d_desc) (void)hipFree(S.d_desc);
     if (S.d_angles) (void)hipFree(S.d_angles);
+    if (S.d_stats) (void)hipFree(S.d_stats);
     if (S.h_angles) (void)hipHostFree(S.h_angles);
     if (S.h_desc) (void)hipHostFree(S.h_desc);
   }
@@ -736,7 +777,7 @@
   if (n > 0) {
     ASD_HIP_CHECK(ctx, hipMemcpyAsync(fe->d_kps, fe->h_kps, (size_t)n * sizeof(short4), hipMemcpyHostToDevice, st));
     hipLaunchKernelGGL(k_angle_patch, dim3((n + 3) / 4), dim3(256), 0, st, P, fe->d_pyr, fe->d_blur, fe->d_kps, n,
-                       S.d_angles, S.d_patches);
+                       S.d_angles, S.d_patches, S.d_stats);
     ASD_HIP_CHECK(ctx, hipGetLastError());
     ASD_HIP_CHECK(ctx, hipMemcpyAsync(S.h_angles, S.d_angles, (size_t)n * sizeof(float), hipMemcpyDeviceToHost, st));
   }
@@ -745,12 +786,12 @@
   return ASD_OK;
 }
 
-static int extract_back_enqueue(asd_ctx* ctx, ExtractSlot& S, int n, hipStream_t st) {
+static int extract_back_enqueue(asd_ctx* ctx, ExtractSlot& S, int n, hipStream_t st, bool host_desc) {
   ASD_HIP_CHECK(ctx, hipStreamWaitEvent(st, S.ev_front, 0));
   if (S.h_range) *S.h_range = 0;
-  const int rc = asdnet_forward_device(ctx, S.d_patches, n, S.d_desc, st, S.h_range);
+  const int rc = asdnet_forward_device(ctx, S.d_patches, n, S.d_desc, st, S.h_range, S.d_stats);
   if (rc != ASD_OK) return rc;
-  ASD_HIP_CHECK(ctx, hipMemcpyAsync(S.h_desc, S.d_desc, (size_t)n * 128 * sizeof(float), hipMemcpyDeviceToHost, st));
+  if (host_desc) ASD_HIP_CHECK(ctx, hipMemcpyAsync(S.h_desc, S.d_desc, (size_t)n * 128 * sizeof(float), hipMemcpyDeviceToHost, st));
   ASD_HIP_CHECK(ctx, hipEventRecord(S.ev_end, st));
   return ASD_OK;
 }
@@ -789,7 +830,7 @@
   ExtractSlot& S = fe->slot0;
   if (!S.d_patches) {
     S.d_patches = ctx->d_patches; S.d_desc = ctx->d_desc;
-    S.d_angles = fe->d_angles; S.h_angles = fe->h_angles; S.h_desc = fe->h_desc;
+    S.d_angles = fe->d_angles; S.h_angles = fe->h_angles; S.h_desc = fe->h_desc; S.d_stats = fe->d_stats;
     S.h_range = reinterpret_cast<int*>(fe->h_angles + ctx->cfg.max_patches);
   }
   if ((rc = slot_events(ctx, S)) != ASD_OK) return rc;
@@ -802,9 +843,11 @@
   ctx->patches_n = n;
   ctx->last_n = n;
   ctx->d_desc_last = S.d_desc;
+  ctx->h_desc_last = S.h_desc;
+  ctx->desc_last_view = ~0ull;
   ctx->d_pyr_view = nullptr;
   if (n == 0) return ASD_OK;
-  if ((rc = extract_back_enqueue(ctx, S, n, ctx->stream)) != ASD_OK) return rc;
+  if ((rc = extract_back_enqueue(ctx, S, n, ctx->stream, true)) != ASD_OK) return rc;
   return extract_finish(ctx, S, n, kps, desc);
 }
 
@@ -877,7 +920,7 @@
       ax->cv.wait(l, [&] { return ax->stop || (ax->back_next == seq && !ax->hold_back); });
       if (ax->stop) return;
     }
-    if (rc == ASD_OK && n > 0) rc = extract_back_enqueue(ctx, S, n, ctx->stream_x);
+    if (rc == ASD_OK && n > 0) rc = extract_back_enqueue(ctx, S, n, ctx->stream_x, ctx->host_desc);
     if (timing) {
       const auto w3 = std::chrono::steady_clock::now();
       auto us = [](auto a, auto b) { return std::chrono::duration<double, std::micro>(b - a).count(); };
@@ -1024,6 +1067,8 @@
   if (a->job.rc != ASD_OK) { *rc = a->job.rc; return nullptr; }
   ctx->last_n = a->job.n;
   ctx->d_desc_last = ax->slots[a->slot].d_desc;
+  ctx->h_desc_last = ax->slots[a->slot].h_desc;
+  ctx->desc_last_view = ax->waited - 1;
   ctx->d_pyr_view = ctx->keep_pyramid ? ax->slots[a->slot].d_pyr_keep : nullptr;
   *rc = ASD_OK;
   return a;
@@ -1036,8 +1081,37 @@
   if (!a) return rc;
   const int n = a->job.n;
   memcpy(kps, a->kps.data(), (size_t)n * sizeof(asd_keypoint));
-  memcpy(desc, ctx->ax->slots[a->slot].h_desc, (size_t)n * 128 * sizeof(float));
+  ExtractSlot& S = ctx->ax->slots[a->slot];
+  if (!ctx->host_desc && n > 0) {
+    ASD_HIP_CHECK(ctx, hipMemcpyAsync(S.h_desc, S.d_desc, (size_t)n * 128 * sizeof(float), hipMemcpyDeviceToHost, ctx->stream));
+    ASD_HIP_CHECK(ctx, hipStreamSynchronize(ctx->stream));
+  }
+  memcpy(desc, S.h_desc, (size_t)n * 128 * sizeof(float));
   *n_out = n;
+  return ASD_OK;
+}
+
+int asd_extract_host_descriptors(asd_ctx* ctx, int32_t on) {
+  if (!ctx) return ASD_ERR_INVALID;
+  if (asd_extractor_busy(ctx, "asd_extract_host_descriptors")) return ASD_ERR_INVALID;
+  ctx->host_desc = on != 0;
+  return ASD_OK;
+}
+int32_t asd_extract_host_descriptors_enabled(const asd_ctx* ctx) { return ctx && ctx->host_desc ? 1 : 0; }
+
+int asd_extract_fetch_descriptors(asd_ctx* ctx, float* desc) {
+  if (!ctx || !desc) return ASD_ERR_INVALID;
+  if (!ctx->d_desc_last) { ctx->set_error("asd_extract_fetch_descriptors: no extraction has completed on this context yet"); return ASD_ERR_INVALID; }
+  if (ctx->desc_last_view != ~0ull && !asd_extract_view_valid(ctx, ctx->desc_last_view)) {
+    ctx->set_error("asd_extract_fetch_descriptors: the view waited for last is no longer valid (%d further submissions have been made)", kSlots);
+    return ASD_ERR_INVALID;
+  }
+  const int n = ctx->last_n;
+  if (n == 0) return ASD_OK;
+  (void)hipSetDevice(ctx->cfg.device);
+  ASD_HIP_CHECK(ctx, hipMemcpyAsync(ctx->h_desc_last, ctx->d_desc_last, (size_t)n * 128 * sizeof(float), hipMemcpyDeviceToHost, ctx->stream));
+  ASD_HIP_CHECK(ctx, hipStreamSynchronize(ctx->stream));
+  memcpy(desc, ctx->h_desc_last, (size_t)n * 128 * sizeof(float));
   return ASD_OK;
 }
 
@@ -1047,7 +1121,7 @@
   AsyncJob* a = wait_oldest(ctx, &rc);
   if (!a) return rc;
   *kps = a->kps.data();
-  *desc = ctx->ax->slots[a->slot].h_desc;
+  *desc = ctx->host_desc ? ctx->ax->slots[a->slot].h_desc : nullptr;
   *n_out = a->job.n;
   return ASD_OK;
 }
@@ -1094,6 +1168,26 @@
   }
   *n_out = n;
   return ASD_OK;
+}
+
+int asd_debug_front_stats(asd_ctx* ctx, int32_t capacity, float* front, float* ref, int32_t* n_out) {
+  if (!ctx || !ctx->fe || !front || !ref || !n_out || capacity < 0) return ASD_ERR_INVALID;
+  if (asd_extractor_busy(ctx, "asd_debug_front_stats")) return ASD_ERR_INVALID;
+  const int n = std::min(ctx->patches_n, (int)capacity);
+  *n_out = n;
+  if (n == 0) return ASD_OK;
+  (void)hipSetDevice(ctx->cfg.device);
+  float* d_ref = nullptr;
+  ASD_HIP_CHECK(ctx, hipMalloc(&d_ref, (size_t)n * 2 * sizeof(float)));
+  int rc = asdnet_patch_stats(ctx, ctx->d_patches, n, d_ref, ctx->stream);
+  if (rc == ASD_OK && (hipMemcpyAsync(ref, d_ref, (size_t)n * 2 * sizeof(float), hipMemcpyDeviceToHost, ctx->stream) != hipSuccess ||
+                       hipMemcpyAsync(front, ctx->fe->d_stats, (size_t)n * 2 * sizeof(float), hipMemcpyDeviceToHost, ctx->stream) != hipSuccess ||
+                       hipStreamSynchronize(ctx->stream) != hipSuccess)) {
+    ctx->set_error("asd_debug_front_stats: copy failed");
+    rc = ASD_ERR_HIP;
+  }
+  (void)hipFree(d_ref);
+  return rc;
 }
 
 int asd_get_patches(asd_ctx* ctx, int32_t capacity, uint8_t* out, int32_t* n_out) {
diff --git a/asd-slam_amd/host/asd_adapters.hpp b/asd-slam_amd/host/asd_adapters.hpp
--- a/asd-slam_amd/host/asd_adapters.hpp
+++ b/asd-slam_amd/host/asd_adapters.hpp
@@ -99,6 +99,12 @@
 inline int FrameAssignFeaturesToGrid(Context& c, FrameView& F, bool adopt_last_extract = true) {
   return asd_frame_set(c.get(), F.slot, F.mvKeysUn.data(), adopt_last_extract ? nullptr : F.mDescriptors.data(), F.N(),
                        F.mnMinX, F.mnMaxX, F.mnMinY, F.mnMaxY);
+}
+
+inline int FrameFetchDescriptors(Context& c, FrameView& F) {
+  F.mDescriptors.resize((size_t)F.N() * ASD_DESC_DIM);
+  if (F.N() == 0) return 0;
+  return asd_extract_fetch_descriptors(c.get(), F.mDescriptors.data()) == ASD_OK ? 0 : -1;
 }
 
 class ORBmatcher {
diff --git a/asd-slam_amd/host/track_loop.cpp b/asd-slam_amd/host/track_loop.cpp
--- a/asd-slam_amd/host/track_loop.cpp
+++ b/asd-slam_amd/host/track_loop.cpp
@@ -32,6 +32,7 @@
   std::vector<uint8_t> dm_ok;
   double dm_ms = 0.0;
   long dm_calls = 0;
+  int host_desc_was = -1, host_desc_was_r = -1;
   asd_ctx* ctx_r = nullptr;
   std::vector<const uint8_t*> d_frames_r;
   float mb = 0.f, mbf = 0.f;
@@ -101,6 +102,8 @@
   h->kf_interval = kf_interval; h->lookahead = lookahead;
   h->kps.resize(1 << 13);
   h->desc_sync.resize((size_t)(1 << 13) * 128);
+  const int32_t was = asd_extract_host_descriptors_enabled(ctx);
+  if (asd_extract_host_descriptors(ctx, 0) == ASD_OK) h->host_desc_was = was;
   return h;
 }
 
@@ -128,6 +131,12 @@
   if (!h || !ctx_right || !d_frames_right || !(mb > 0) || !(mbf > 0) || !h->pending.empty()) return ASD_ERR_INVALID;
   int rc;
   if ((rc = asd_extract_keep_pyramid(h->ctx, 1)) != ASD_OK || (rc = asd_extract_keep_pyramid(ctx_right, 1)) != ASD_OK) return rc;
+  if (h->ctx_r != ctx_right) {
+    if (h->ctx_r && h->host_desc_was_r >= 0) (void)asd_extract_host_descriptors(h->ctx_r, h->host_desc_was_r);
+    h->host_desc_was_r = -1;
+    const int32_t was = asd_extract_host_descriptors_enabled(ctx_right);
+    if (asd_extract_host_descriptors(ctx_right, 0) == ASD_OK) h->host_desc_was_r = was;
+  }
   h->ctx_r = ctx_right;
   h->d_frames_r.clear();
   for (size_t i = 0; i < h->d_frames.size(); ++i) h->d_frames_r.push_back(static_cast<const uint8_t*>(d_frames_right[i]));
@@ -178,6 +187,8 @@
     h->pending.pop_front();
   }
   (void)collect_ba(h, nullptr, -1);
+  if (h->host_desc_was >= 0) (void)asd_extract_host_descriptors(h->ctx, h->host_desc_was);
+  if (h->ctx_r && h->host_desc_was_r >= 0) (void)asd_extract_host_descriptors(h->ctx_r, h->host_desc_was_r);
   if (getenv("ASD_TIMING") && h->steps)
   {
     fprintf(stderr, "[track_loop] steps %ld  extract wait %.3f ms/step  local BA %.3f ms/step (+ %.3f ms/step putting its problem together on the host)\n", h->steps,
diff --git a/include/asd_slam.h b/include/asd_slam.h
--- a/include/asd_slam.h
+++ b/include/asd_slam.h
@@ -73,6 +73,9 @@
                        int32_t height, int32_t stride, int32_t n_features_override);
 int asd_extract_wait(asd_ctx* ctx, asd_keypoint* kps, float* desc, int32_t* n_out);
 int asd_extract_wait_view(asd_ctx* ctx, const asd_keypoint** kps, const float** desc, int32_t* n_out);
+int asd_extract_host_descriptors(asd_ctx* ctx, int32_t on);
+int32_t asd_extract_host_descriptors_enabled(const asd_ctx* ctx);
+int asd_extract_fetch_descriptors(asd_ctx* ctx, float* desc);
 uint64_t asd_extract_last_view(const asd_ctx* ctx);
 int32_t asd_extract_view_valid(asd_ctx* ctx, uint64_t view_id);
 
```

After: 1238. -1.5%, worse.
